# DrorT/demucs

Hardware: NVIDIA B200
Metric: htdemucs audio-seconds separated per second (higher is better)
Workload: dtype f32 (bf16 hi/lo split operands, 3 tcgen05 products, fp32 accumulate)

## Files before the change

### demucs_b200/_lib.py

```python
from __future__ import annotations

import ctypes as C
import os
import subprocess
import typing as tp

HERE = os.path.dirname(os.path.abspath(__file__))
CSRC = os.path.join(HERE, "csrc")
LIB_PATH = os.path.join(HERE, "libdemucs_b200.so")
SOURCES = ["api.cu", "spectral.cu", "gemm_simt.cu", "gemm_tc.cu", "gemm_tc_b16x3.cu", "gemm_tc_b16.cu", "norm.cu", "dconv.cu", "attention.cu", "attention_tc.cu", "attention_b16.cu",
           "ola.cu", "audio.cu", "hdemucs.cu"]
NVCC_FLAGS = ["-gencode", "arch=compute_100a,code=sm_100a", "-lineinfo", "-O3", "-std=c++17",
              "-Xcompiler", "-fPIC", "--use_fast_math=false"]

BD_MAX_TAPS = 9
A_NONE, A_GN_GELU, A_ITEM_AFFINE = 0, 1, 2
ACT_NONE, ACT_GELU, ACT_GLU = 0, 1, 2
MATH_FP32, MATH_TF32, MATH_TF32X3, MATH_BF16X3, MATH_BF16 = 0, 1, 2, 3, 4


class KernelError(RuntimeError):
    pass


class GemmDesc(C.Structure):
    _fields_ = [
        ("M", C.c_int), ("N", C.c_int), ("K", C.c_int),
        ("Cin", C.c_int), ("taps", C.c_int),
        ("I1", C.c_int), ("I0", C.c_int),
        ("m1", C.c_int), ("m0", C.c_int), ("J1", C.c_int), ("J0", C.c_int),
        ("d1", C.c_int * BD_MAX_TAPS), ("d0", C.c_int * BD_MAX_TAPS),
        ("xs_b", C.c_longlong), ("xs_1", C.c_longlong), ("xs_0", C.c_longlong), ("xs_c", C.c_longlong),
        ("x", C.c_void_p), ("w", C.c_void_p), ("bias", C.c_void_p),
        ("a_mode", C.c_int), ("a_stats", C.c_void_p), ("a_stats_stride", C.c_int),
        ("a_gamma", C.c_void_p), ("a_beta", C.c_void_p),
        ("e_stats", C.c_void_p), ("e_gamma", C.c_void_p), ("e_beta", C.c_void_p),
        ("act", C.c_int), ("rowbias", C.c_void_p), ("rowbias_period", C.c_int),
        ("resid", C.c_void_p), ("scale", C.c_void_p), ("addend", C.c_void_p),
        ("out", C.c_void_p), ("os_b", C.c_longlong), ("os_1", C.c_longlong), ("os_0", C.c_longlong),
        ("convt", C.c_int), ("O0", C.c_int), ("oc_split", C.c_int), ("oc_stride", C.c_longlong),
        ("stats_out", C.c_void_p), ("stat_div", C.c_int), ("stat_mul", C.c_int), ("stat_mod", C.c_int),
        ("math", C.c_int), ("w16_hi", C.c_void_p), ("w16_lo", C.c_void_p), ("x_bf16", C.c_int), ("out_bf16", C.c_int),
    ]


_P, _I, _LL, _D, _F = C.c_void_p, C.c_int, C.c_longlong, C.c_double, C.c_float
SIGNATURES: tp.Dict[str, tp.List] = {
    "bd_stft_cac": [_P, _P, _P, _P, _P, _I, _I, _I, _P],
    "bd_finalize_item_norm": [_P, _P, _I, _D, _D, _P],
    "bd_istft_frames": [_P, _P, _P, _P, _P, _I, _I, _I, _P],
    "bd_istft_ola": [_P, _P, _P, _P, _P, _P, _I, _I, _I, _I, _I, _P],
    "bd_ola_combine": [_P, _P, _P, _P, _I, _I, _I, _I, _I, _P],
    "bd_conv_gemm": [C.POINTER(GemmDesc), _P],
    "bd_conv_gemm_arm": [C.POINTER(GemmDesc)],
    "bd_finalize_group_stats": [_P, _P, _I, _D, _P],
    "bd_dconv_tail": [_P, _P, _P, _P, _P, _P, _LL, _I, _LL, _I, _P],
    "bd_encoder_conv0": [_P, _I, _P, _I, _P, _P, _P, _I, _I, _I, _I, _I, _I, _I, _P],
    "bd_dconv_conv3": [_P, _P, _P, _P, _I, _P, _LL, _I, _I, _LL, _I, _I, _I, _P],
    "bd_dconv_expand_stats": [_P, _I, _I, _P, _P, _P, _P, _P, _P, _P, _LL, _I, _LL, _I, _P],
    "bd_dconv_expand_update": [_P, _I, _I, _P, _P, _P, _P, _P, _P, _P, _P, _P, _P, _LL, _I, _LL, _I, _I, _P],
    "bd_gn_gelu_apply": [_P, _P, _P, _P, _LL, _I, _LL, _I, _P],
    "bd_layer_norm": [_P, _P, _P, _P, _P, _I, _LL, _I, _I, _P],
    "bd_attention_bf16": [_P, _P, _P, _P, _I, _I, _I, _I, _I, _I, _I, _I, _P],
    "bd_item_stats": [_P, _P, _I, _LL, _P],
    "bd_group_norm_apply": [_P, _P, _P, _P, _I, _LL, _I, _P],
    "bd_attention_workspace": [_I, _I, _I, _I, _I],
    "bd_attention": [_P, _P, _P, _P, _I, _I, _I, _I, _I, _I, _I, _I, _I, _P, _P],
    "bd_overlap_add": [_P, _P, _P, _I, _I, _I, _I, _I, _I, _I, _LL, _LL, _LL, _LL, _LL, _P, _F, _I, _P],
    "bd_gather_segments": [_P, _P, _I, _I, _LL, _LL, _LL, _I, _I, _I, _I, _I, _P],
    "bd_gn_stats": [_P, _P, _I, _LL, _I, _I, _P],
    "bd_gn_act": [_P, _P, _P, _P, _P, _P, _I, _LL, _LL, _LL, _I, _I, _I, _LL, _P],
    "bd_lstm_frame": [_P, _P, _I, _LL, _I, _I, _I, _I, _P],
    "bd_lstm_unframe_add": [_P, _P, _P, _I, _LL, _I, _I, _I, _I, _P],
    "bd_lstm_bidir": [_P, _P, _P, _P, _I, _I, _I, _P],
    "bd_local_state": [_P, _P, _P, _I, _I, _I, _I, _P],
    "bd_convert_channels": [_P, _P, _I, _I, _I, _LL, _P],
    "bd_resample_frac": [_P, _P, _P, _I, _I, _I, _LL, _LL, _I, _I, _I, _P],
    "bd_absmax": [_P, _P, _LL, _P],
    "bd_clip_pcm": [_P, _P, _I, _LL, _I, _P, _I, _P],
}
VALUE_CALLS = {"bd_attention_workspace"}
EXPORTS = ["bd_last_error", "bd_version"] + list(SIGNATURES)

_lib: tp.Optional[C.CDLL] = None


def build(verbose: bool = False, force: bool = False) -> str:
    import hashlib
    from concurrent.futures import ThreadPoolExecutor
    srcs = [os.path.join(CSRC, s) for s in SOURCES if os.path.exists(os.path.join(CSRC, s))]
    headers = [os.path.join(os.path.dirname(HERE), "include", "demucs_b200.h")]
    headers += sorted(os.path.join(CSRC, f) for f in os.listdir(CSRC) if f.endswith(".cuh"))
    flags = [f for f in NVCC_FLAGS if not f.startswith("--use_fast_math")]
    flags += os.environ.get("BD_NVCC_DEFS", "").split()
    base = hashlib.sha256(" ".join(flags).encode())
    for dep in headers:
        with open(dep, "rb") as f:
            base.update(f.read())
    nvcc = os.environ.get("NVCC", "/usr/local/cuda/bin/nvcc")
    objdir = os.path.join(CSRC, ".obj")
    os.makedirs(objdir, exist_ok=True)
    total = base.copy()
    jobs = []
    for src in srcs:
        d = base.copy()
        with open(src, "rb") as f:
            data = f.read()
        d.update(data)
        total.update(data)
        obj = os.path.join(objdir, os.path.basename(src)[:-3] + ".o")
        jobs.append((src, obj, d.hexdigest()))
    stamp_path = LIB_PATH + ".stamp"
    stamp = total.hexdigest()
    if not force and os.path.exists(LIB_PATH) and os.path.exists(stamp_path):
        with open(stamp_path) as f:
            if f.read().strip() == stamp:
                return LIB_PATH

    def compile_one(job):
        src, obj, digest = job
        if not force and os.path.exists(obj) and os.path.exists(obj + ".stamp"):
            with open(obj + ".stamp") as f:
                if f.read().strip() == digest:
                    return ""
        cmd = [nvcc] + flags + (["-Xptxas=-v"] if verbose else []) + ["-c", "-o", obj, src]
        res = subprocess.run(cmd, capture_output=True, text=True)
        if res.returncode != 0:
            raise KernelError(f"nvcc failed on {src}:\n{res.stdout}\n{res.stderr}")
        with open(obj + ".stamp", "w") as f:
            f.write(digest)
        return res.stderr

    with ThreadPoolExecutor(max_workers=min(len(jobs), os.cpu_count() or 4)) as pool:
        logs = list(pool.map(compile_one, jobs))
    if verbose:
        print("\n".join(logs))
    res = subprocess.run([nvcc] + flags + ["-shared", "-o", LIB_PATH] + [j[1] for j in jobs], capture_output=True, text=True)
    if res.returncode != 0:
        raise KernelError(f"link failed:\n{res.stdout}\n{res.stderr}")
    with open(stamp_path, "w") as f:
        f.write(stamp)
    return LIB_PATH


def lib() -> C.CDLL:
    global _lib
    if _lib is None:
        if not os.path.exists(LIB_PATH):
            raise KernelError(
                f"{LIB_PATH} is missing: run `python -c 'import __graft_entry__ as g; g.build()'` "
                "(demucs_b200 has no CPU or PyTorch fallback path)")
        handle = C.CDLL(LIB_PATH)
        handle.bd_last_error.restype = C.c_char_p
        handle.bd_last_error.argtypes = []
        handle.bd_version.restype = C.c_int
        for name, args in SIGNATURES.items():
            fn = getattr(handle, name)
            fn.restype = C.c_longlong if name in VALUE_CALLS else C.c_int
            fn.argtypes = args
        _lib = handle
    return _lib


TEST_HOOK: tp.Optional[tp.Callable] = None


def call(name: str, *args) -> None:
    if TEST_HOOK is not None:
        return TEST_HOOK(name, *args)
    rc = getattr(lib(), name)(*args)
    if rc != 0:
        raise KernelError(f"{name} failed ({rc}): {lib().bd_last_error().decode()}")


def call_value(name: str, *args) -> int:
    if TEST_HOOK is not None:
        return TEST_HOOK(name, *args)
    return int(getattr(lib(), name)(*args))


def ptr(t) -> tp.Optional[int]:
    return None if t is None else t.data_ptr()
```

### demucs_b200/csrc/gemm_tc.cu

```cuda
#include "gemm_tc_impl.cuh"

int bd_tc_launch_bf16x3(int tbk, int tbn, const bd_gemm_desc& d, const TileGeom& g, int items, cudaStream_t st);
int bd_tc_launch_bf16(int tbk, int tbn, const bd_gemm_desc& d, const TileGeom& g, int items, cudaStream_t st);
int bd_tc_launch_bf16d(int tbk, int tbn, const bd_gemm_desc& d, const TileGeom& g, int items, cudaStream_t st);

namespace {
int pow2_ceil(int v) {
  int p = 1;
  while (p < v) p <<= 1;
  return p;
}
}

bool bd_conv_gemm_tc_eligible(const bd_gemm_desc& d) {
  if (d.a_mode != BD_A_NONE || d.xs_c != 1 || d.m1 != 1) return false;
  if (!(d.m0 == 1 || (d.m0 == 4 && d.J0 % 4 == 0))) return false;
  if (d.Cin % 16 != 0 || d.N < 16 || d.K < 16 || d.M < 128 || d.taps > BD_MAX_TAPS) return false;
  if (d.x_bf16) {
    if (d.math != BD_MATH_BF16 || d.Cin % 64 != 0) return false;
    if (d.xs_0 % 8 != 0 || (d.J1 > 1 && d.xs_1 % 8 != 0) || d.xs_b % 8 != 0) return false;
  }
  if (d.xs_0 % 4 != 0 || (d.J1 > 1 && d.xs_1 % 4 != 0) || d.xs_b % 4 != 0) return false;
  if (((uintptr_t)d.x & 15) || ((uintptr_t)d.w & 15)) return false;
  if (d.math == BD_MATH_BF16X3 || d.math == BD_MATH_BF16) {
    if (!d.w16_hi || ((uintptr_t)d.w16_hi & 15) || d.K % 8 != 0) return false;
    if (d.math == BD_MATH_BF16X3 && (!d.w16_lo || ((uintptr_t)d.w16_lo & 15))) return false;
  }
  if (d.stats_out && d.stat_mod == 1 && !(d.I1 == 1 && d.I0 == d.stat_div)) return false;
  return true;
}

namespace {

TileGeom tile_geometry(const bd_gemm_desc& d) {
  TileGeom g;
  g.R0 = (d.I0 >= 128 || d.I1 == 1) ? 128 : (pow2_ceil(d.I0) > 128 ? 128 : pow2_ceil(d.I0));
  g.R1 = 128 / g.R0;
  g.log2R0 = 0;
  while ((1 << g.log2R0) < g.R0) ++g.log2R0;
  g.blocks0 = (d.I0 + g.R0 - 1) / g.R0;
  g.blocks1 = (d.I1 + g.R1 - 1) / g.R1;
  g.stride4 = d.m0 == 4;
  g.cpb = 0;
  return g;
}

int tile_width(const bd_gemm_desc& d, const TileGeom& g) {
  static const bool wide_ok = getenv("BD_TC_NO_WIDE") == nullptr;
  static const bool wide_x3 = getenv("BD_TC_NO_WIDE_X3") == nullptr;
  const int items = d.M / (d.I0 * d.I1);
  const bool wide = wide_ok && (d.math != BD_MATH_TF32X3 || wide_x3) && d.N % 256 == 0 &&
                    d.K >= 256 && d.out && !d.convt && !d.oc_split && !d.rowbias && !d.addend && !d.e_stats &&
                    (!d.stats_out || d.stat_mod == 1) && bd_epi_vec_ok(d);
  auto wave_eff = [&](int tile_n) {
    const long long t = (long long)items * g.blocks1 * g.blocks0 * ((d.N + tile_n - 1) / tile_n);
    return (double)t / (double)(((t + 147) / 148) * 148);
  };
  if (wide && wave_eff(256) >= wave_eff(128) - 0.05) return 256;
  return d.N <= 16 ? 16 : d.N <= 32 ? 32 : d.N <= 64 ? 64 : 128;
}

}

static int k_block(const bd_gemm_desc& d, int tbn) {
  if (d.x_bf16) return 64;
  if (d.math == BD_MATH_BF16X3 || d.math == BD_MATH_BF16) return d.Cin % 32 == 0 ? 32 : 16;
  return (tbn == 256 || d.math == BD_MATH_TF32X3 || d.Cin % 32 != 0) ? 16 : 32;
}

int bd_conv_gemm_tc_tile(const bd_gemm_desc& d) {
  if (!bd_conv_gemm_tc_eligible(d) || d.M % ((long long)d.I0 * d.I1) != 0) return 0;
  const int tbn = tile_width(d, tile_geometry(d));
  return 1000 * k_block(d, tbn) + tbn;
}

int bd_conv_gemm_tc(const bd_gemm_desc* dp, void* stream, int* handled) {
  const bd_gemm_desc& d = *dp;
  *handled = 0;
  if (!bd_conv_gemm_tc_eligible(d)) return BD_OK;
  BD_REQUIRE(d.act != BD_ACT_GLU || d.N % 2 == 0, "bd_conv_gemm: GLU needs even N");
  BD_REQUIRE(d.M % ((long long)d.I0 * d.I1) == 0, "bd_conv_gemm: M not a multiple of I1*I0");
  TileGeom g = tile_geometry(d);
  const int items = d.M / (d.I0 * d.I1);
  const int tbn = tile_width(d, g);
  const int tbk = k_block(d, tbn);
  g.cpb = d.Cin / tbk;
  const cudaStream_t st = (cudaStream_t)stream;
  int rc;
  switch (d.math) {
    case BD_MATH_BF16X3: rc = bd_tc_launch_bf16x3(tbk, tbn, d, g, items, st); break;
    case BD_MATH_BF16:
      rc = d.x_bf16 ? bd_tc_launch_bf16d(tbk, tbn, d, g, items, st) : bd_tc_launch_bf16(tbk, tbn, d, g, items, st);
      break;
    case BD_MATH_TF32X3:
      rc = tbn == 256 ? launch_tc_persist<16, 256, BD_TC_TF32X3>(d, g, items, st)
                      : launch_tc_width<16, BD_TC_TF32X3>(tbn, d, g, items, st);
      break;
    default:
      rc = tbn == 256 ? launch_tc_persist<16, 256, BD_TC_TF32>(d, g, items, st)
           : tbk == 32 ? launch_tc_width<32, BD_TC_TF32>(tbn, d, g, items, st)
                       : launch_tc_width<16, BD_TC_TF32>(tbn, d, g, items, st);
      break;
  }
  *handled = 1;
  return rc;
}
```

### demucs_b200/csrc/gemm_tc_impl.cuh

```cuda
#pragma once
#include <cuda.h>
#include <stdlib.h>
#include "gemm_epilogue.cuh"

enum { BD_TC_TF32 = 0, BD_TC_TF32X3 = 1, BD_TC_BF16X3 = 2, BD_TC_BF16 = 3, BD_TC_BF16D = 4 };

struct TileGeom {
  int R0, R1;
  int log2R0;
  int blocks0, blocks1;
  int cpb;
  int stride4;
};

namespace {

constexpr int TBM = 128;


struct RowInfo {
  long long obase;
  int i0;
  int rb_row;
  float e_mean, e_rstd;
  int pad0, pad1;
};

constexpr uint32_t kSpinLimit = 1u << 26;

__device__ __forceinline__ uint32_t smem_u32(const void* p) { return (uint32_t)__cvta_generic_to_shared(p); }

__device__ __forceinline__ void mbar_init(uint64_t* bar, uint32_t count) {
  asm volatile("mbarrier.init.shared::cta.b64 [%0], %1;" ::"r"(smem_u32(bar)), "r"(count));
}
__device__ __forceinline__ void mbar_arrive(uint64_t* bar) {
  asm volatile("mbarrier.arrive.shared::cta.b64 _, [%0];" ::"r"(smem_u32(bar)) : "memory");
}
__device__ __forceinline__ void mbar_expect_tx(uint64_t* bar, uint32_t bytes) {
  asm volatile("mbarrier.arrive.expect_tx.shared::cta.b64 _, [%0], %1;" ::"r"(smem_u32(bar)), "r"(bytes) : "memory");
}
__device__ __forceinline__ void mbar_wait(uint64_t* bar, uint32_t parity) {
  uint32_t done = 0, spins = 0;
  while (true) {
    asm volatile(
        "{\n\t.reg .pred p;\n\t"
        "mbarrier.try_wait.parity.shared::cta.b64 p, [%1], %2;\n\t"
        "selp.u32 %0, 1, 0, p;\n\t}"
        : "=r"(done)
        : "r"(smem_u32(bar)), "r"(parity)
        : "memory");
    if (done) return;
    if (++spins > kSpinLimit) __trap();
  }
}
__device__ __forceinline__ void mbar_wait_parked(uint64_t* bar, uint32_t parity) {
  uint32_t done = 0, spins = 0;
  while (true) {
    asm volatile(
        "{\n\t.reg .pred p;\n\t"
        "mbarrier.try_wait.parity.shared::cta.b64 p, [%1], %2, %3;\n\t"
        "selp.u32 %0, 1, 0, p;\n\t}"
        : "=r"(done)
        : "r"(smem_u32(bar)), "r"(parity), "r"(1000)
        : "memory");
    if (done) return;
    if (++spins > kSpinLimit) __trap();
  }
}
__device__ __forceinline__ void mbar_wait_relaxed(uint64_t* bar, uint32_t parity) {
  uint32_t done = 0, spins = 0;
  while (true) {
    asm volatile(
        "{\n\t.reg .pred p;\n\t"
        "mbarrier.try_wait.parity.shared::cta.b64 p, [%1], %2;\n\t"
        "selp.u32 %0, 1, 0, p;\n\t}"
        : "=r"(done)
        : "r"(smem_u32(bar)), "r"(parity)
        : "memory");
    if (done) return;
    __nanosleep(64);
    if (++spins > kSpinLimit) __trap();
  }
}
__device__ __forceinline__ void tma_load_4d(const CUtensorMap* map, uint64_t* bar, void* dst, int c0, int c1, int c2,
                                            int c3) {
  asm volatile(
      "cp.async.bulk.tensor.4d.shared::cluster.global.mbarrier::complete_tx::bytes [%0], [%1, {%3, %4, %5, %6}], [%2];"
      ::"r"(smem_u32(dst)), "l"((uint64_t)map), "r"(smem_u32(bar)), "r"(c0), "r"(c1), "r"(c2), "r"(c3)
      : "memory");
}
__device__ __forceinline__ void tma_load_5d(const CUtensorMap* map, uint64_t* bar, void* dst, int c0, int c1, int c2,
                                            int c3, int c4) {
  asm volatile(
      "cp.async.bulk.tensor.5d.shared::cluster.global.mbarrier::complete_tx::bytes [%0], [%1, {%3, %4, %5, %6, %7}], "
      "[%2];"
      ::"r"(smem_u32(dst)), "l"((uint64_t)map), "r"(smem_u32(bar)), "r"(c0), "r"(c1), "r"(c2), "r"(c3), "r"(c4)
      : "memory");
}
__device__ __forceinline__ void tma_load_2d(const CUtensorMap* map, uint64_t* bar, void* dst, int c0, int c1) {
  asm volatile(
      "cp.async.bulk.tensor.2d.shared::cluster.global.mbarrier::complete_tx::bytes [%0], [%1, {%3, %4}], [%2];"
      ::"r"(smem_u32(dst)), "l"((uint64_t)map), "r"(smem_u32(bar)), "r"(c0), "r"(c1)
      : "memory");
}
__device__ __forceinline__ void tcgen05_commit(uint64_t* bar) {
  asm volatile("tcgen05.commit.cta_group::1.mbarrier::arrive::one.shared::cluster.b64 [%0];" ::"r"(smem_u32(bar))
               : "memory");
}
__device__ __forceinline__ void tcgen05_fence_after() { asm volatile("tcgen05.fence::after_thread_sync;" ::: "memory"); }
__device__ __forceinline__ void tcgen05_fence_before() { asm volatile("tcgen05.fence::before_thread_sync;" ::: "memory"); }

__device__ __forceinline__ void umma_tf32(uint32_t tmem_d, uint64_t adesc, uint64_t bdesc, uint32_t idesc, uint32_t accumulate) {
  asm volatile(
      "{\n\t.reg .pred p;\n\t"
      "setp.ne.b32 p, %4, 0;\n\t"
      "tcgen05.mma.cta_group::1.kind::tf32 [%0], %1, %2, %3, p;\n\t}"
      ::"r"(tmem_d), "l"(adesc), "l"(bdesc), "r"(idesc), "r"(accumulate)
      : "memory");
}

__device__ __forceinline__ void umma_bf16(uint32_t tmem_d, uint64_t adesc, uint64_t bdesc, uint32_t idesc, uint32_t accumulate) {
  asm volatile(
      "{\n\t.reg .pred p;\n\t"
      "setp.ne.b32 p, %4, 0;\n\t"
      "tcgen05.mma.cta_group::1.kind::f16 [%0], %1, %2, %3, p;\n\t}"
      ::"r"(tmem_d), "l"(adesc), "l"(bdesc), "r"(idesc), "r"(accumulate)
      : "memory");
}

template <int TBK>
__device__ __forceinline__ uint64_t make_kmajor_desc(const void* smem) {
  uint64_t desc = (uint64_t)((smem_u32(smem) & 0x3FFFF) >> 4);
  desc |= (uint64_t)((8 * TBK * 4) >> 4) << 32;
  desc |= (uint64_t)1 << 46;
  desc |= (uint64_t)(TBK == 32 ? 2 : 4) << 61;
  return desc;
}
template <int TBK>
__device__ __forceinline__ uint64_t make_kmajor_desc16(const void* smem, int sbo) {
  uint64_t desc = (uint64_t)((smem_u32(smem) & 0x3FFFF) >> 4);
  desc |= (uint64_t)(sbo >> 4) << 32;
  desc |= (uint64_t)1 << 46;
  desc |= (uint64_t)(TBK == 64 ? 2 : TBK == 32 ? 4 : 6) << 61;
  return desc;
}
__host__ __device__ constexpr uint32_t make_idesc_bf16(int M, int N) {
  return (1u << 4) | (1u << 7) | (1u << 10) | ((uint32_t)(N >> 3) << 17) | ((uint32_t)(M >> 4) << 24);
}
__device__ __forceinline__ uint32_t pack_bf16(float a, float b) {
  uint32_t r;
  asm("cvt.rn.bf16x2.f32 %0, %1, %2;" : "=r"(r) : "f"(b), "f"(a));
  return r;
}
__host__ __device__ constexpr uint32_t make_idesc_tf32(int M, int N) {
  return (1u << 4) | (2u << 7) | (2u << 10) | ((uint32_t)(N >> 3) << 17) | ((uint32_t)(M >> 4) << 24);
}

__device__ __forceinline__ void tmem_ld32(uint32_t taddr, uint32_t* r) {
  asm volatile(
      "tcgen05.ld.sync.aligned.32x32b.x32.b32 "
      "{%0, %1, %2, %3, %4, %5, %6, %7, %8, %9, %10, %11, %12, %13, %14, %15, "
      "%16, %17, %18, %19, %20, %21, %22, %23, %24, %25, %26, %27, %28, %29, %30, %31}, [%32];"
      : "=r"(r[0]), "=r"(r[1]), "=r"(r[2]), "=r"(r[3]), "=r"(r[4]), "=r"(r[5]), "=r"(r[6]), "=r"(r[7]), "=r"(r[8]),
        "=r"(r[9]), "=r"(r[10]), "=r"(r[11]), "=r"(r[12]), "=r"(r[13]), "=r"(r[14]), "=r"(r[15]), "=r"(r[16]),
        "=r"(r[17]), "=r"(r[18]), "=r"(r[19]), "=r"(r[20]), "=r"(r[21]), "=r"(r[22]), "=r"(r[23]), "=r"(r[24]),
        "=r"(r[25]), "=r"(r[26]), "=r"(r[27]), "=r"(r[28]), "=r"(r[29]), "=r"(r[30]), "=r"(r[31])
      : "r"(taddr));
  asm volatile("tcgen05.wait::ld.sync.aligned;" ::: "memory");
}

__device__ __forceinline__ float rn_tf32(float x) {
  uint32_t u;
  asm("cvt.rna.tf32.f32 %0, %1;" : "=r"(u) : "f"(x));
  return __uint_as_float(u);
}

__device__ __forceinline__ void tmem_ld16(uint32_t taddr, uint32_t* r) {
  asm volatile(
      "tcgen05.ld.sync.aligned.32x32b.x16.b32 "
      "{%0, %1, %2, %3, %4, %5, %6, %7, %8, %9, %10, %11, %12, %13, %14, %15}, [%16];"
      : "=r"(r[0]), "=r"(r[1]), "=r"(r[2]), "=r"(r[3]), "=r"(r[4]), "=r"(r[5]), "=r"(r[6]), "=r"(r[7]), "=r"(r[8]),
        "=r"(r[9]), "=r"(r[10]), "=r"(r[11]), "=r"(r[12]), "=r"(r[13]), "=r"(r[14]), "=r"(r[15])
      : "r"(taddr));
  asm volatile("tcgen05.wait::ld.sync.aligned;" ::: "memory");
}

__device__ __forceinline__ float sigmoid_fast(float x) {
  float e, r;
  asm("ex2.approx.ftz.f32 %0, %1;" : "=f"(e) : "f"(-1.44269504088896340736f * x));
  asm("rcp.approx.ftz.f32 %0, %1;" : "=f"(r) : "f"(1.0f + e));
  return r;
}
__device__ __forceinline__ float4 lds128(uint32_t a) {
  float4 v;
  asm volatile("ld.shared.v4.f32 {%0, %1, %2, %3}, [%4];" : "=f"(v.x), "=f"(v.y), "=f"(v.z), "=f"(v.w) : "r"(a));
  return v;
}

template <int ACT, bool E, bool RES, bool ROWB, bool CT, int WC, int RB>
__device__ __forceinline__ void epi_fast_rows(const bd_gemm_desc& d, uint32_t stage_s, uint32_t rinfo_s, int lane, int n0w,
                                              float& ssum, float& ssq) {
  constexpr int LDT = WC + 4;
  constexpr int CG = WC / 4 < 32 ? WC / 4 : 32;
  constexpr int RPI = 32 / CG;
  const int cg = lane % CG, rsub = lane / CG;
  const int n = n0w + 4 * cg;
  const bool col_ok = n < d.N;
  const int nc = col_ok ? n : 0;
  const float4 bias = d.bias ? ldg4(d.bias + nc) : make_float4(0.f, 0.f, 0.f, 0.f);
  float4 gam = make_float4(1.f, 1.f, 1.f, 1.f), bet = make_float4(0.f, 0.f, 0.f, 0.f);
  if (E) {
    gam = ldg4(d.e_gamma + nc);
    bet = ldg4(d.e_beta + nc);
  }
  const int no = ACT == BD_ACT_GLU ? nc >> 1 : nc;
  float4 scl = make_float4(1.f, 1.f, 1.f, 1.f);
  if (RES && d.scale) {
    if (ACT == BD_ACT_GLU) {
      const float2 t = ldg2(d.scale + no);
      scl.x = t.x; scl.y = t.y;
    } else {
      scl = ldg4(d.scale + no);
    }
  }
  int rr = 0;
  long long colofs = no;
  if (CT) {
    const int cout = d.N >> 2;
    rr = nc / cout;
    colofs = (long long)rr * d.os_0 + (nc - rr * cout);
    rr -= d.convt == 1 ? 2 : 0;
  }
  const long long outo = colofs;
  const float* resp = RES ? d.resid + colofs : nullptr;
  const float* addp = CT && d.addend ? d.addend + colofs : nullptr;
  const float* rbp = ROWB ? d.rowbias + no : nullptr;
  const int rb_ld = ACT == BD_ACT_GLU ? d.N >> 1 : d.N;
  const uint32_t st_lane = stage_s + (uint32_t)(rsub * LDT + 4 * cg) * 4u;
  const uint32_t ri_lane = rinfo_s + (uint32_t)rsub * 32u;
#pragma unroll 1
  for (int it = 0; it < 32 / RPI; it += RB) {
    long long ob[RB];
    bool ok[RB];
    float mean[RB], rstd[RB];
    float4 res[RB];
#pragma unroll
    for (int u = 0; u < RB; ++u) {
      const uint32_t ra = ri_lane + (uint32_t)((it + u) * RPI) * 32u;
      uint32_t w0, w1, w2, w3;
      asm volatile("ld.shared.v4.u32 {%0, %1, %2, %3}, [%4];" : "=r"(w0), "=r"(w1), "=r"(w2), "=r"(w3) : "r"(ra));
      ob[u] = (long long)(((unsigned long long)w1 << 32) | w0);
      ok[u] = (int)w2 >= 0 && col_ok;
      if (CT) ok[u] = ok[u] && (unsigned)(4 * (int)w2 + rr) < (unsigned)d.O0;
      if (ROWB || CT) res[u] = make_float4(0.f, 0.f, 0.f, 0.f);
      if (ROWB && ok[u]) {
        if (ACT == BD_ACT_GLU) {
          const float2 t = ldg2(rbp + (size_t)w3 * rb_ld);
          res[u].x = t.x; res[u].y = t.y;
        } else {
          res[u] = ldg4(rbp + (size_t)w3 * rb_ld);
        }
      }
      if (CT && addp && ok[u]) res[u] = ldg4(addp + ob[u]);
      if (E) asm volatile("ld.shared.v2.f32 {%0, %1}, [%2];" : "=f"(mean[u]), "=f"(rstd[u]) : "r"(ra + 16));
      if (RES) {
        res[u] = make_float4(0.f, 0.f, 0.f, 0.f);
        if (ok[u]) {
          if (ACT == BD_ACT_GLU) {
            const float2 t = ldg2(resp + ob[u]);
            res[u].x = t.x; res[u].y = t.y;
          } else {
            res[u] = ldg4(resp + ob[u]);
          }
        }
      }
    }
#pragma unroll
    for (int u = 0; u < RB; ++u) {
      float4 v = lds128(st_lane + (uint32_t)((it + u) * RPI * LDT) * 4u);
      v.x += bias.x; v.y += bias.y; v.z += bias.z; v.w += bias.w;
      if (E) {
        v.x = fmaf((v.x - mean[u]) * rstd[u], gam.x, bet.x);
        v.y = fmaf((v.y - mean[u]) * rstd[u], gam.y, bet.y);
        v.z = fmaf((v.z - mean[u]) * rstd[u], gam.z, bet.z);
        v.w = fmaf((v.w - mean[u]) * rstd[u], gam.w, bet.w);
      }
      if (ACT == BD_ACT_GLU) {
        float2 o2 = make_float2(v.x * sigmoid_fast(v.y), v.z * sigmoid_fast(v.w));
        if (ROWB) {
          o2.x += res[u].x;
          o2.y += res[u].y;
        }
        if (RES) {
          o2.x = fmaf(scl.x, o2.x, res[u].x);
          o2.y = fmaf(scl.y, o2.y, res[u].y);
        }
        if (ok[u]) {
          bd_store_out2(d, outo + ob[u], o2);
          ssum += o2.x + o2.y;
          ssq = fmaf(o2.x, o2.x, fmaf(o2.y, o2.y, ssq));
        }
      } else {
        if (ACT == BD_ACT_GELU) {
          v.x = bd_gelu(v.x); v.y = bd_gelu(v.y); v.z = bd_gelu(v.z); v.w = bd_gelu(v.w);
        }
        if (RES) {
          v.x = fmaf(scl.x, v.x, res[u].x); v.y = fmaf(scl.y, v.y, res[u].y);
          v.z = fmaf(scl.z, v.z, res[u].z); v.w = fmaf(scl.w, v.w, res[u].w);
        }
        if (ROWB || CT) {
          v.x += res[u].x; v.y += res[u].y; v.z += res[u].z; v.w += res[u].w;
        }
        if (ok[u]) {
          bd_store_out4(d, outo + ob[u], v);
          ssum += (v.x + v.y) + (v.z + v.w);
          ssq = fmaf(v.x, v.x, fmaf(v.y, v.y, fmaf(v.z, v.z, fmaf(v.w, v.w, ssq))));
        }
      }
    }
  }
}

__device__ __forceinline__ int epi_fast_id(const bd_gemm_desc& d, bool vec, bool row_stats) {
  if (!vec || row_stats || !d.out || d.oc_split) return -1;
  const bool e = d.e_stats != nullptr, r = d.resid != nullptr;
  if (d.convt) return (d.act == BD_ACT_GELU && !e && !r && !d.rowbias) ? 6 : -1;
  if (d.addend) return -1;
  if (d.rowbias) return (d.act == BD_ACT_GLU && !e && !r) ? 5 : -1;
  if (d.act == BD_ACT_NONE && !e) return r ? 1 : 0;
  if (d.act == BD_ACT_GELU && !e && !r) return 2;
  if (d.act == BD_ACT_GLU && !e && !r) return 3;
  if (d.act == BD_ACT_GLU && e && r) return 4;
  return -1;
}

#ifndef BD_TC_EPI_GROUPS
#define BD_TC_EPI_GROUPS 4
#endif
template <int TBK, int TBN, int MODE>
struct PCfg {
  static constexpr bool kX3 = MODE == BD_TC_TF32X3;
  static constexpr bool kB16 = MODE == BD_TC_BF16X3 || MODE == BD_TC_BF16 || MODE == BD_TC_BF16D;
  static constexpr bool kDirect = MODE == BD_TC_BF16D;
  static constexpr bool kSplit = MODE != BD_TC_TF32 && !kDirect;
  static constexpr int kBParts = MODE == BD_TC_BF16X3 ? 2 : 1;
  static constexpr int kPGroups = (MODE == BD_TC_TF32X3 || MODE == BD_TC_BF16X3) ? 2 : BD_TC_EPI_GROUPS;
  static constexpr int kSplitWarp0 = kB16 ? 2 : 4;
  static constexpr int kSplitWarps = MODE == BD_TC_BF16 ? 2 : 4;
  static constexpr int kEpiWarp0 = kSplit ? kSplitWarp0 + kSplitWarps : 4;
  static constexpr int kThreads = 32 * kEpiWarp0 + 128 * kPGroups;
  static constexpr int kTileBytesA = TBM * TBK * (kDirect ? 2 : 4);
  static constexpr int kTileBytesB = kB16 ? TBN * TBK * 2 : TBN * TBK * 4;
  static constexpr int kStageBytesA = (kX3 ? 2 : 1) * kTileBytesA;
  static constexpr int kStageBytesB = (kX3 ? 2 : kBParts) * kTileBytesB;
  static constexpr int kTxBytes = kTileBytesA + (kB16 ? kBParts : 1) * kTileBytesB;
  static constexpr bool kTileSplit = TBN <= 32;
  static constexpr int kNAcc = kTileSplit ? kPGroups : 2;
  static constexpr int kHalves = TBN > 128 ? 2 : 1;
  static constexpr int kWarpCols = kTileSplit ? TBN : (TBN / kHalves) / kPGroups;
  static constexpr int kStagingBytes = 4 * kPGroups * 32 * (kWarpCols + 4) * 4;
  static constexpr int kTailBytes = 512 + 128 * kPGroups * 32;
  static constexpr int kBudget = 227 * 1024 - 1024 - kTailBytes - kStagingBytes;
  static constexpr int kStagesRaw = kBudget / (kStageBytesA + kStageBytesB);
  static constexpr int kStages = kStagesRaw > (kTileSplit ? 16 : 8) ? (kTileSplit ? 16 : 8) : kStagesRaw;
  static constexpr int kSmemBytes = kStages * (kStageBytesA + kStageBytesB) + kStagingBytes + 1024 + kTailBytes;
  static constexpr int kTmemCols = kNAcc * TBN < 32 ? 32 : kNAcc * TBN;
};

template <int TBK, int TBN, int MODE>
__global__ void __launch_bounds__((PCfg<TBK, TBN, MODE>::kThreads), 1) conv_gemm_tc_persist_kernel(const __grid_constant__ CUtensorMap map_a,
                                                                            const __grid_constant__ CUtensorMap map_b,
                                                                            const __grid_constant__ CUtensorMap map_b_lo,
                                                                            const bd_gemm_desc d, const TileGeom g,
                                                                            int ntiles, int ntn) {
  using C_ = PCfg<TBK, TBN, MODE>;
  constexpr bool X3 = C_::kX3, B16 = C_::kB16, SPLIT = C_::kSplit;
  constexpr int kPGroups = C_::kPGroups;
  constexpr int kTileBytesA = C_::kTileBytesA, kTileBytesB = C_::kTileBytesB;
  constexpr int kStages = C_::kStages, kStageBytesA = C_::kStageBytesA, kStageBytesB = C_::kStageBytesB;
  constexpr int kTmemCols = C_::kTmemCols;
  constexpr int WC = C_::kWarpCols;
  constexpr int CW = WC < 32 ? WC : 32;
  extern __shared__ uint8_t smem_raw[];
  uint8_t* smem = reinterpret_cast<uint8_t*>(((uintptr_t)smem_raw + 1023) & ~(uintptr_t)1023);
  uint8_t* sA = smem;
  uint8_t* sB = smem + kStages * kStageBytesA;
  float* staging = reinterpret_cast<float*>(sB + kStages * kStageBytesB);
  uint64_t* full_bar = reinterpret_cast<uint64_t*>(reinterpret_cast<uint8_t*>(staging) + C_::kStagingBytes);
  uint64_t* empty_bar = full_bar + kStages;
  constexpr int kNAcc = C_::kNAcc;
  constexpr bool kTileSplit = C_::kTileSplit;
  constexpr int NH = C_::kHalves;
  uint64_t* tmem_full = empty_bar + kStages;
  uint64_t* tmem_empty = tmem_full + kNAcc;
  uint64_t* conv_bar = tmem_empty + kNAcc;
  uint32_t* tmem_slot = reinterpret_cast<uint32_t*>(conv_bar + kStages);

  const int warp = threadIdx.x >> 5, lane = threadIdx.x & 31;
  const int nkb = d.taps * g.cpb;

  if (threadIdx.x == 0) {
    for (int s = 0; s < kStages; ++s) {
      mbar_init(&full_bar[s], 1);
      mbar_init(&empty_bar[s], 1);
      mbar_init(&conv_bar[s], 32 * C_::kSplitWarps);
    }
    for (int a = 0; a < kNAcc; ++a) {
      mbar_init(&tmem_full[a], 1);
      mbar_init(&tmem_empty[a], kTileSplit ? 4 : 4 * kPGroups);
    }
    asm volatile("fence.mbarrier_init.release.cluster;" ::: "memory");
  }
  if (warp == 1) {
    asm volatile("tcgen05.alloc.cta_group::1.sync.aligned.shared::cta.b32 [%0], %1;" ::"r"(smem_u32(tmem_slot)),
                 "r"(kTmemCols));
    asm volatile("tcgen05.relinquish_alloc_permit.cta_group::1.sync.aligned;" ::);
  }
  tcgen05_fence_before();
  __syncthreads();
  tcgen05_fence_after();
  const uint32_t tmem_base = *tmem_slot;

  auto decode = [&](int tile, int& b, int& i0s, int& i1s, int& n0) {
    const int nb = tile % ntn;
    int r = tile / ntn;
    const int blk0 = r % g.blocks0;
    r /= g.blocks0;
    const int blk1 = r % g.blocks1;
    b = r / g.blocks1;
    i0s = blk0 * g.R0;
    i1s = blk1 * g.R1;
    n0 = nb * TBN;
  };

  if (warp == 0) {
    if (lane == 0) {
      long long kbg = 0;
      for (int tile = blockIdx.x; tile < ntiles; tile += gridDim.x) {
        int b, i0s, i1s, n0;
        decode(tile, b, i0s, i1s, n0);
        int tap = 0, cb = 0;
        for (int kb = 0; kb < nkb; ++kb, ++kbg) {
          const int s = (int)(kbg % kStages);
          const uint32_t ph = (uint32_t)((kbg / kStages) & 1);
          mbar_wait_parked(&empty_bar[s], ph ^ 1);
          mbar_expect_tx(&full_bar[s], C_::kTxBytes);
          if (g.stride4) {
            const int d0 = d.d0[tap];
            tma_load_5d(&map_a, &full_bar[s], sA + s * kStageBytesA, cb * TBK, d0 & 3, i0s + (d0 >> 2), i1s + d.d1[tap], b);
          } else {
            tma_load_4d(&map_a, &full_bar[s], sA + s * kStageBytesA, cb * TBK, i0s + d.d0[tap], i1s + d.d1[tap], b);
          }
          tma_load_2d(&map_b, &full_bar[s], sB + s * kStageBytesB, tap * d.Cin + cb * TBK, n0);
          if constexpr (MODE == BD_TC_BF16X3)
            tma_load_2d(&map_b_lo, &full_bar[s], sB + s * kStageBytesB + kTileBytesB, tap * d.Cin + cb * TBK, n0);
          if (++cb == g.cpb) {
            cb = 0;
            ++tap;
          }
        }
      }
    }
  } else if (warp == 1) {
    if (lane == 0) {
      constexpr uint32_t idesc = B16 ? make_idesc_bf16(TBM, TBN) : make_idesc_tf32(TBM, TBN);
      long long kbg = 0;
      int tcount = 0;
      for (int tile = blockIdx.x; tile < ntiles; tile += gridDim.x, ++tcount) {
        const int a = tcount % kNAcc;
        mbar_wait_parked(&tmem_empty[a], (uint32_t)(((tcount / kNAcc) & 1) ^ 1));
        tcgen05_fence_after();
        const uint32_t acc = tmem_base + (uint32_t)(a * TBN);
        for (int kb = 0; kb < nkb; ++kb, ++kbg) {
          const int s = (int)(kbg % kStages);
          const uint32_t ph = (uint32_t)((kbg / kStages) & 1);
          mbar_wait_parked(SPLIT ? &conv_bar[s] : &full_bar[s], ph);
          tcgen05_fence_after();
          if constexpr (B16) {
            const uint64_t a_hi = make_kmajor_desc16<TBK>(sA + s * kStageBytesA, C_::kDirect ? 8 * TBK * 2 : 8 * TBK * 4);
            const uint64_t a_lo = make_kmajor_desc16<TBK>(sA + s * kStageBytesA + 8 * TBK * 2, 8 * TBK * 4);
            const uint64_t b_hi = make_kmajor_desc16<TBK>(sB + s * kStageBytesB, 8 * TBK * 2);
            const uint64_t b_lo = make_kmajor_desc16<TBK>(sB + s * kStageBytesB + kTileBytesB, 8 * TBK * 2);
#pragma unroll
            for (int k = 0; k < TBK / 16; ++k) {
              if constexpr (MODE == BD_TC_BF16X3) {
                umma_bf16(acc, a_lo + 2 * k, b_hi + 2 * k, idesc, (kb | k) != 0);
                umma_bf16(acc, a_hi + 2 * k, b_lo + 2 * k, idesc, 1);
                umma_bf16(acc, a_hi + 2 * k, b_hi + 2 * k, idesc, 1);
              } else {
                umma_bf16(acc, a_hi + 2 * k, b_hi + 2 * k, idesc, (kb | k) != 0);
              }
            }
          } else {
          const uint64_t adesc = make_kmajor_desc<TBK>(sA + s * kStageBytesA);
          const uint64_t bdesc = make_kmajor_desc<TBK>(sB + s * kStageBytesB);
#pragma unroll
          for (int k = 0; k < TBK / 8; ++k) {
            if constexpr (X3) {
              const uint64_t alo = make_kmajor_desc<TBK>(sA + s * kStageBytesA + kTileBytesA);
              const uint64_t blo = make_kmajor_desc<TBK>(sB + s * kStageBytesB + kTileBytesB);
              umma_tf32(acc, alo + 2 * k, bdesc + 2 * k, idesc, (kb | k) != 0);
              umma_tf32(acc, adesc + 2 * k, blo + 2 * k, idesc, 1);
              umma_tf32(acc, adesc + 2 * k, bdesc + 2 * k, idesc, 1);
            } else {
              umma_tf32(acc, adesc + 2 * k, bdesc + 2 * k, idesc, (kb | k) != 0);
            }
          }
          }
          tcgen05_commit(&empty_bar[s]);
        }
        tcgen05_commit(&tmem_full[a]);
      }
    }
  } else if (SPLIT && warp >= C_::kSplitWarp0 && warp < C_::kSplitWarp0 + C_::kSplitWarps) {
    const int et = threadIdx.x - 32 * C_::kSplitWarp0;
    long long kbg = 0;
    if constexpr (B16) {
      constexpr int RB = TBK * 4, RH = TBK * 2;
      constexpr int GB = 8 * RB;
      constexpr int SW = C_::kSplitWarps;
      constexpr int NG = (TBM / 8) / SW;
      const int sw = warp - C_::kSplitWarp0, r = lane >> 2, q = lane & 3;
      const int xin = (r * RB >> 7) & (RB / 16 - 1);
      const int xout = (r * RH >> 7) & (RH / 16 - 1);
      (void)et;
      for (int tile = blockIdx.x; tile < ntiles; tile += gridDim.x) {
        for (int kb = 0; kb < nkb; ++kb, ++kbg) {
          const int s = (int)(kbg % kStages);
          mbar_wait(&full_bar[s], (uint32_t)((kbg / kStages) & 1));
          uint8_t* base = sA + s * kStageBytesA;
#pragma unroll
          for (int i0 = 0; i0 < NG; i0 += 4) {
          float4 v[4][TBK == 32 ? 2 : 1];
#pragma unroll
          for (int i = 0; i < 4; ++i) {
            const uint8_t* gp = base + (sw + SW * (i0 + i)) * GB + r * RB;
            if constexpr (TBK == 32) {
              v[i][0] = *reinterpret_cast<const float4*>(gp + (((2 * q) ^ xin) << 4));
              v[i][1] = *reinterpret_cast<const float4*>(gp + (((2 * q + 1) ^ xin) << 4));
            } else {
              v[i][0] = *reinterpret_cast<const float4*>(gp + ((q ^ xin) << 4));
            }
          }
          __syncwarp();
#pragma unroll
          for (int i = 0; i < 4; ++i) {
            uint8_t* gp = base + (sw + SW * (i0 + i)) * GB + r * RH;
            uint32_t hi[TBK == 32 ? 4 : 2], lo[TBK == 32 ? 4 : 2];
#pragma unroll
            for (int j = 0; j < (TBK == 32 ? 2 : 1); ++j) {
              const float4 x = v[i][j];
              const uint32_t h0 = pack_bf16(x.x, x.y), h1 = pack_bf16(x.z, x.w);
              hi[2 * j] = h0;
              hi[2 * j + 1] = h1;
              lo[2 * j] = lo[2 * j + 1] = 0u;
              if constexpr (MODE == BD_TC_BF16X3) {
                lo[2 * j] = pack_bf16(x.x - __uint_as_float(h0 << 16), x.y - __uint_as_float(h0 & 0xffff0000u));
                lo[2 * j + 1] = pack_bf16(x.z - __uint_as_float(h1 << 16), x.w - __uint_as_float(h1 & 0xffff0000u));
              }
            }
            if constexpr (TBK == 32) {
              uint8_t* dst = gp + ((q ^ xout) << 4);
              *reinterpret_cast<uint4*>(dst) = make_uint4(hi[0], hi[1], hi[2], hi[3]);
              if constexpr (MODE == BD_TC_BF16X3) *reinterpret_cast<uint4*>(dst + 8 * RH) = make_uint4(lo[0], lo[1], lo[2], lo[3]);
            } else {
              uint8_t* dst = gp + (((q >> 1) ^ xout) << 4) + ((q & 1) << 3);
              *reinterpret_cast<uint2*>(dst) = make_uint2(hi[0], hi[1]);
              if constexpr (MODE == BD_TC_BF16X3) *reinterpret_cast<uint2*>(dst + 8 * RH) = make_uint2(lo[0], lo[1]);
            }
          }
          }
          asm volatile("fence.proxy.async.shared::cta;" ::: "memory");
          mbar_arrive(&conv_bar[s]);
        }
      }
    } else {
    for (int tile = blockIdx.x; tile < ntiles; tile += gridDim.x) {
      for (int kb = 0; kb < nkb; ++kb, ++kbg) {
        const int s = (int)(kbg % kStages);
        mbar_wait(&full_bar[s], (uint32_t)((kbg / kStages) & 1));
        auto split = [&](uint8_t* base, int tile_bytes) {
          float4* hi = reinterpret_cast<float4*>(base);
          float4* lo = reinterpret_cast<float4*>(base + tile_bytes);
#pragma unroll 4
          for (int i = et; i < tile_bytes / 16; i += 128) {
            const float4 x = hi[i];
            const float4 h = make_float4(rn_tf32(x.x), rn_tf32(x.y), rn_tf32(x.z), rn_tf32(x.w));
            hi[i] = h;
            lo[i] = make_float4(x.x - h.x, x.y - h.y, x.z - h.z, x.w - h.w);
          }
        };
        split(sA + s * kStageBytesA, kTileBytesA);
        split(sB + s * kStageBytesB, kTileBytesB);
        asm volatile("fence.proxy.async.shared::cta;" ::: "memory");
        mbar_arrive(&conv_bar[s]);
      }
    }
    }
  } else if (warp >= C_::kEpiWarp0) {
    const int quarter = warp & 3, ew = warp - C_::kEpiWarp0, grp = ew >> 2;
    const int cbase = kTileSplit ? 0 : grp * WC;
    const bool row_stats = d.stats_out && d.stat_mod != 1;
    const bool vec = bd_epi_vec_ok(d);
    const int fast = epi_fast_id(d, vec, row_stats);
    constexpr int LDT = WC + 4;
    float* stage = staging + (size_t)ew * 32 * LDT;
    RowInfo* rinfo = reinterpret_cast<RowInfo*>(((uintptr_t)(tmem_slot + 4) + 31) & ~(uintptr_t)31) + ew * 32;
    int tcount = 0;
    for (int tile = blockIdx.x; tile < ntiles; tile += gridDim.x, ++tcount) {
      if (kTileSplit && tcount % kPGroups != grp) continue;
      int b, i0s, i1s, n0;
      decode(tile, b, i0s, i1s, n0);
      const int a = tcount % kNAcc;
      const int r = quarter * 32 + lane;
      const int i0 = i0s + (r & (g.R0 - 1)), i1 = i1s + (r >> g.log2R0);
      const bool row_ok = i0 < d.I0 && i1 < d.I1;
      const long long m = ((long long)b * d.I1 + i1) * d.I0 + i0;
      EpiRow er;
      er.obase = 0; er.i0 = 0; er.rb_row = 0; er.e_mean = 0.f; er.e_rstd = 1.f;
      if (row_ok) {
        er.i0 = i0;
        er.obase = (long long)b * d.os_b + (long long)i1 * d.os_1 +
                   (long long)(d.convt ? 4 * i0 - (d.convt == 1 ? 2 : 0) : i0) * d.os_0;
        if (d.rowbias) er.rb_row = (int)((unsigned)m % (unsigned)d.rowbias_period);
        if (d.e_stats) {
          const int sl = bd_stat_slab(d, m);
          er.e_mean = __ldg(d.e_stats + 2 * (size_t)sl);
          er.e_rstd = __ldg(d.e_stats + 2 * (size_t)sl + 1);
        }
      }
      const int my_slab = (d.stats_out && row_ok) ? bd_stat_slab(d, m) : -1;
      float ssum = 0.f, ssq = 0.f;
      if (d.resid && row_ok && !d.convt && !d.oc_split) {
        const int c0 = n0 + cbase;
        if (c0 < d.N) {
          const float* pf = d.resid + er.obase + (d.act == BD_ACT_GLU ? c0 >> 1 : c0);
          asm volatile("prefetch.global.L2 [%0];" ::"l"(pf));
        }
      }
      for (int half = 0; half < NH; ++half) {
      const int n0h = n0 + 128 * half;
      if (half == 0) {
        mbar_wait_relaxed(&tmem_full[a], (uint32_t)((tcount / kNAcc) & 1));
        tcgen05_fence_after();
      } else {
        __syncwarp();
      }
      const bool last_half = half == NH - 1;
      const uint32_t acc = tmem_base + (uint32_t)(a * TBN + 128 * half + cbase) + ((uint32_t)(quarter * 32) << 16);
      if (vec) {
        rinfo[lane].obase = er.obase;
        rinfo[lane].i0 = row_ok ? er.i0 : -1;
        rinfo[lane].rb_row = er.rb_row;
        rinfo[lane].e_mean = er.e_mean;
        rinfo[lane].e_rstd = er.e_rstd;
        for (int c0 = 0; c0 < WC; c0 += CW) {
          if (n0h + cbase + c0 >= d.N) break;
          uint32_t v[CW];
          if constexpr (CW == 32) tmem_ld32(acc + c0, v); else tmem_ld16(acc + c0, v);
#pragma unroll
          for (int j = 0; j < CW; j += 4)
            *reinterpret_cast<float4*>(stage + lane * LDT + c0 + j) =
                make_float4(__uint_as_float(v[j]), __uint_as_float(v[j + 1]), __uint_as_float(v[j + 2]),
                            __uint_as_float(v[j + 3]));
        }
        tcgen05_fence_before();
        __syncwarp();
        if (lane == 0 && last_half) mbar_arrive(&tmem_empty[a]);
        if (fast >= 0) {
          const uint32_t st_s = smem_u32(stage), ri_s = smem_u32(rinfo);
          const int n0w = n0h + cbase;
          constexpr int FRB = kPGroups >= 4 ? 2 : 4;
          switch (fast) {
            case 0: epi_fast_rows<BD_ACT_NONE, false, false, false, false, WC, FRB>(d, st_s, ri_s, lane, n0w, ssum, ssq); break;
            case 1: epi_fast_rows<BD_ACT_NONE, false, true, false, false, WC, FRB>(d, st_s, ri_s, lane, n0w, ssum, ssq); break;
            case 2: epi_fast_rows<BD_ACT_GELU, false, false, false, false, WC, FRB>(d, st_s, ri_s, lane, n0w, ssum, ssq); break;
            case 3: epi_fast_rows<BD_ACT_GLU, false, false, false, false, WC, FRB>(d, st_s, ri_s, lane, n0w, ssum, ssq); break;
            case 4: epi_fast_rows<BD_ACT_GLU, true, true, false, false, WC, FRB>(d, st_s, ri_s, lane, n0w, ssum, ssq); break;
            case 5: epi_fast_rows<BD_ACT_GLU, false, false, true, false, WC, FRB>(d, st_s, ri_s, lane, n0w, ssum, ssq); break;
            default: epi_fast_rows<BD_ACT_GELU, false, false, false, true, WC, FRB>(d, st_s, ri_s, lane, n0w, ssum, ssq); break;
          }
          __syncwarp();
        } else {
        constexpr int CG = WC / 4 < 32 ? WC / 4 : 32;
        constexpr int RPI = 32 / CG;
        constexpr int RB = kPGroups >= 4 ? 2 : 4;
        const int cg = lane % CG, rsub = lane / CG;
        const int n = n0h + cbase + 4 * cg;
        const bool col_ok = n < d.N;
        EpiCol ecol;
        if (col_ok) ecol = bd_epi_cols4(d, n);
        for (int it = 0; it < 32 / RPI; it += RB) {
          EpiRow row[RB];
          EpiMem mem[RB];
          bool ok[RB];
#pragma unroll
          for (int u = 0; u < RB; ++u) {
            const int rloc = (it + u) * RPI + rsub;
            const uint32_t ra = smem_u32(&rinfo[rloc]);
            uint32_t w0, w1, w2, w3, w4, w5;
            asm volatile("ld.shared.v4.u32 {%0, %1, %2, %3}, [%4];" : "=r"(w0), "=r"(w1), "=r"(w2), "=r"(w3) : "r"(ra));
            asm volatile("ld.shared.v2.u32 {%0, %1}, [%2];" : "=r"(w4), "=r"(w5) : "r"(ra + 16));
            row[u].obase = (long long)(((unsigned long long)w1 << 32) | w0);
            row[u].i0 = (int)w2;
            row[u].rb_row = (int)w3;
            row[u].e_mean = __uint_as_float(w4);
            row[u].e_rstd = __uint_as_float(w5);
            ok[u] = row[u].i0 >= 0 && col_ok;
            if (ok[u]) mem[u] = bd_epi_fetch4(d, row[u], ecol);
          }
#pragma unroll
          for (int u = 0; u < RB; ++u) {
            const int rloc = (it + u) * RPI + rsub;
            float rs = 0.f, rq = 0.f;
            if (ok[u]) {
              const float4 acc4 = *reinterpret_cast<const float4*>(stage + rloc * LDT + 4 * cg);
              bd_epi_finish4(d, row[u], ecol, acc4, mem[u], rs, rq);
            }
            if (row_stats) {
              __syncwarp();
              *reinterpret_cast<float2*>(stage + rloc * LDT + 2 * cg) = make_float2(rs, rq);
            } else {
              ssum += rs;
              ssq += rq;
            }
          }
        }
        if (row_stats) {
          __syncwarp();
          float rs = 0.f, rq = 0.f;
#pragma unroll
          for (int c = 0; c < CG; ++c) {
            const float2 t = *reinterpret_cast<const float2*>(stage + lane * LDT + 2 * c);
            rs += t.x;
            rq += t.y;
          }
          if (my_slab >= 0) {
            atomicAdd(&d.stats_out[2 * (size_t)my_slab], (double)rs);
            atomicAdd(&d.stats_out[2 * (size_t)my_slab + 1], (double)rq);
          }
        }
        __syncwarp();
        }
      } else {
        for (int c0 = 0; c0 < WC; c0 += CW) {
          if (n0h + cbase + c0 >= d.N) break;
          uint32_t v[CW];
          if constexpr (CW == 32) tmem_ld32(acc + c0, v); else tmem_ld16(acc + c0, v);
          if (row_ok) {
#pragma unroll
            for (int j = 0; j < CW; ++j) {
              const int n = n0h + cbase + c0 + j;
              if (n < d.N) {
                float st;
                if (bd_epi_apply(d, er, n, __uint_as_float(v[j]), __uint_as_float(v[(j + 1) % CW]), st)) {
                  ssum += st;
                  ssq = fmaf(st, st, ssq);
                }
              }
            }
          }
        }
        tcgen05_fence_before();
        __syncwarp();
        if (lane == 0 && last_half) mbar_arrive(&tmem_empty[a]);
        if (row_stats && row_ok) {
          atomicAdd(&d.stats_out[2 * (size_t)my_slab], (double)ssum);
          atomicAdd(&d.stats_out[2 * (size_t)my_slab + 1], (double)ssq);
        }
      }
      }
      if (d.stats_out && d.stat_mod == 1) {
        const double ds = bd_warp_sum_d((double)ssum), dq = bd_warp_sum_d((double)ssq);
        if (lane == 0) {
          const int sl = bd_stat_slab(d, (long long)b * d.I1 * d.I0 + i0s);
          atomicAdd(&d.stats_out[2 * (size_t)sl], ds);
          atomicAdd(&d.stats_out[2 * (size_t)sl + 1], dq);
        }
      }
    }
  }
  tcgen05_fence_before();
  __syncthreads();
  if (warp == 1) {
    tcgen05_fence_after();
    asm volatile("tcgen05.dealloc.cta_group::1.sync.aligned.b32 %0, %1;" ::"r"(tmem_base), "r"(kTmemCols));
  }
}

typedef CUresult (*EncodeTiledFn)(CUtensorMap*, CUtensorMapDataType, cuuint32_t, void*, const cuuint64_t*,
                                  const cuuint64_t*, const cuuint32_t*, const cuuint32_t*, CUtensorMapInterleave,
                                  CUtensorMapSwizzle, CUtensorMapL2promotion, CUtensorMapFloatOOBfill);

EncodeTiledFn get_encode_fn() {
  static EncodeTiledFn fn = nullptr;
  if (!fn) {
    void* p = nullptr;
    cudaDriverEntryPointQueryResult q;
    if (cudaGetDriverEntryPoint("cuTensorMapEncodeTiled", &p, cudaEnableDefault, &q) != cudaSuccess ||
        q != cudaDriverEntryPointSuccess)
      return nullptr;
    fn = (EncodeTiledFn)p;
  }
  return fn;
}

bool encode(CUtensorMap* map, const void* base, int rank, const cuuint64_t* gdim, const cuuint64_t* gstride_bytes,
            const cuuint32_t* box, int row_bytes, bool bf16 = false) {
  EncodeTiledFn enc = get_encode_fn();
  if (!enc) return false;
  cuuint32_t estr[5] = {1, 1, 1, 1, 1};
  const CUtensorMapSwizzle sw = row_bytes == 128 ? CU_TENSOR_MAP_SWIZZLE_128B
                                : row_bytes == 64 ? CU_TENSOR_MAP_SWIZZLE_64B : CU_TENSOR_MAP_SWIZZLE_32B;
  return enc(map, bf16 ? CU_TENSOR_MAP_DATA_TYPE_BFLOAT16 : CU_TENSOR_MAP_DATA_TYPE_FLOAT32, rank, (void*)base, gdim,
             gstride_bytes, box, estr, CU_TENSOR_MAP_INTERLEAVE_NONE, sw, CU_TENSOR_MAP_L2_PROMOTION_L2_128B,
             CU_TENSOR_MAP_FLOAT_OOB_FILL_NONE) == CUDA_SUCCESS;
}

template <int TBK, int TBN, int MODE>
int launch_tc_persist(const bd_gemm_desc& d, const TileGeom& g, int items, cudaStream_t st) {
  using C_ = PCfg<TBK, TBN, MODE>;
  alignas(64) CUtensorMap map_a, map_b, map_b_lo;
  const long long s0 = d.xs_0, s1 = d.J1 > 1 ? d.xs_1 : s0 * d.J0, sb = items > 1 ? d.xs_b : s1 * d.J1;
  constexpr int ES = C_::kDirect ? 2 : 4;
  cuuint64_t adim[5] = {(cuuint64_t)d.Cin, (cuuint64_t)d.J0, (cuuint64_t)d.J1, (cuuint64_t)items, 1};
  cuuint64_t astr[4] = {(cuuint64_t)s0 * ES, (cuuint64_t)s1 * ES, (cuuint64_t)sb * ES, 0};
  cuuint32_t abox[5] = {(cuuint32_t)TBK, (cuuint32_t)g.R0, (cuuint32_t)g.R1, 1, 1};
  int arank = 4;
  if (g.stride4) {
    arank = 5;
    adim[1] = 4; adim[2] = (cuuint64_t)d.J0 / 4; adim[3] = (cuuint64_t)d.J1; adim[4] = (cuuint64_t)items;
    astr[0] = (cuuint64_t)s0 * ES; astr[1] = (cuuint64_t)s0 * 4 * ES; astr[2] = (cuuint64_t)s1 * ES; astr[3] = (cuuint64_t)sb * ES;
    abox[1] = 1; abox[2] = (cuuint32_t)g.R0; abox[3] = (cuuint32_t)g.R1; abox[4] = 1;
  }
  cuuint64_t bdim[2] = {(cuuint64_t)d.K, (cuuint64_t)d.N};
  cuuint32_t bbox[2] = {(cuuint32_t)TBK, (cuuint32_t)TBN};
  bool ok = encode(&map_a, d.x, arank, adim, astr, abox, TBK * ES, C_::kDirect);
  if constexpr (C_::kB16) {
    cuuint64_t bstr[1] = {(cuuint64_t)d.K * 2};
    ok = ok && encode(&map_b, d.w16_hi, 2, bdim, bstr, bbox, TBK * 2, true);
    ok = ok && encode(&map_b_lo, MODE == BD_TC_BF16X3 ? d.w16_lo : d.w16_hi, 2, bdim, bstr, bbox, TBK * 2, true);
  } else {
    cuuint64_t bstr[1] = {(cuuint64_t)d.K * 4};
    ok = ok && encode(&map_b, d.w, 2, bdim, bstr, bbox, TBK * 4);
    map_b_lo = map_b;
  }
  if (!ok) {
    bd_set_error("bd_conv_gemm_tc: cuTensorMapEncodeTiled failed (M=%d N=%d K=%d Cin=%d J0=%d J1=%d)", d.M, d.N, d.K,
                 d.Cin, d.J0, d.J1);
    return BD_ERR_CUDA;
  }
  static int sms_of[64] = {0};
  int dev = 0;
  cudaGetDevice(&dev);
  if (dev < 0 || dev >= 64) {
    bd_set_error("bd_conv_gemm_tc: device ordinal %d out of range", dev);
    return BD_ERR_ARG;
  }
  if (!sms_of[dev]) {
    cudaError_t e = cudaFuncSetAttribute(conv_gemm_tc_persist_kernel<TBK, TBN, MODE>,
                                         cudaFuncAttributeMaxDynamicSharedMemorySize, C_::kSmemBytes);
    if (e != cudaSuccess) {
      bd_set_error("bd_conv_gemm_tc: cudaFuncSetAttribute: %s", cudaGetErrorString(e));
      return BD_ERR_CUDA;
    }
    int n = 0;
    cudaDeviceGetAttribute(&n, cudaDevAttrMultiProcessorCount, dev);
    sms_of[dev] = n;
  }
  const int sms = sms_of[dev];
  const int ntn = (d.N + TBN - 1) / TBN;
  const long long ntiles = (long long)items * g.blocks1 * g.blocks0 * ntn;
  const int grid = (int)(ntiles < sms ? ntiles : sms);
  conv_gemm_tc_persist_kernel<TBK, TBN, MODE><<<grid, C_::kThreads, C_::kSmemBytes, st>>>(map_a, map_b, map_b_lo, d, g,
                                                                                         (int)ntiles, ntn);
  return bd_check_launch("conv_gemm_tc_persist_kernel");
}

template <int TBK, int MODE>
int launch_tc_width(int tbn, const bd_gemm_desc& d, const TileGeom& g, int items, cudaStream_t st) {
  switch (tbn) {
    case 16: return launch_tc_persist<TBK, 16, MODE>(d, g, items, st);
    case 32: return launch_tc_persist<TBK, 32, MODE>(d, g, items, st);
    case 64: return launch_tc_persist<TBK, 64, MODE>(d, g, items, st);
    case 128: return launch_tc_persist<TBK, 128, MODE>(d, g, items, st);
    default: break;
  }
  bd_set_error("bd_conv_gemm_tc: no kernel for tile width %d", tbn);
  return BD_ERR_ARG;
}

}
```

### demucs_b200/engine.py

```python
from __future__ import annotations

import ctypes as C
import math
import typing as tp

import numpy as np
import torch

from . import _lib
from ._lib import GemmDesc, call, ptr
from .config import HTDemucsConfig
from .weights import check_state_dict

MODES = ("fp32", "tf32", "tf32x3", "strict", "bf16")
_GEMM_MATH = {"fp32": _lib.MATH_FP32, "tf32": _lib.MATH_TF32, "tf32x3": _lib.MATH_TF32X3, "strict": _lib.MATH_BF16X3,
              "bf16": _lib.MATH_BF16}
_ATTN_MATH = dict(_GEMM_MATH)


def _interleave_glu(w: torch.Tensor) -> torch.Tensor:
    half = w.shape[0] // 2
    return torch.stack([w[:half], w[half:]], dim=1).reshape(w.shape).contiguous()


def _sin_embedding_1d(length: int, dim: int, max_period: float) -> torch.Tensor:
    pos = torch.arange(length, dtype=torch.float32)[:, None]
    half = dim // 2
    k = torch.arange(half, dtype=torch.float32)[None, :]
    phase = pos / (max_period ** (k / (half - 1)))
    return torch.cat([torch.cos(phase), torch.sin(phase)], dim=-1)


def _sin_embedding_2d(dim: int, height: int, width: int, max_period: float) -> torch.Tensor:
    half = dim // 2
    div = torch.exp(torch.arange(0.0, half, 2) * -(math.log(max_period) / half))
    pw = torch.arange(0.0, width)[:, None] * div[None, :]
    ph = torch.arange(0.0, height)[:, None] * div[None, :]
    pe = torch.zeros(width, height, dim)
    pe[:, :, 0:half:2] = torch.sin(pw)[:, None, :]
    pe[:, :, 1:half:2] = torch.cos(pw)[:, None, :]
    pe[:, :, half::2] = torch.sin(ph)[None, :, :]
    pe[:, :, half + 1::2] = torch.cos(ph)[None, :, :]
    return pe.reshape(width * height, dim)


def conv_w(w):
    w = w.detach().float()
    co, ci = w.shape[:2]
    return w.reshape(co, ci, -1).permute(0, 2, 1).reshape(co, -1)


def convtr_w(w):
    w = w.detach().float()
    ci, co = w.shape[:2]
    w = w.reshape(ci, co, 2, 4)
    return w.permute(3, 1, 2, 0).reshape(4 * co, 2 * ci)


def convtr_w3(w):
    w = w.detach().float()
    ci, co = w.shape[:2]
    w = w.reshape(ci, co, 8)
    out = torch.zeros(4, co, 3, ci)
    for s_ in range(4):
        out[s_, :, 1] = w[:, :, s_ + 2].t()
        if s_ <= 1:
            out[s_, :, 0] = w[:, :, s_ + 6].t()
        else:
            out[s_, :, 2] = w[:, :, s_ - 2].t()
    return out.reshape(4 * co, 3 * ci)


def pack_dconv(put, packed, state, prefix: str, depth: int, tc_forms: bool, idx=(0, 1, 3, 4, 6)) -> None:
    i_c3, i_n1, i_c1, i_n2, i_ls = idx
    for d in range(depth):
        p = f"{prefix}.dconv.layers.{d}"
        put(f"{p}.w1", conv_w(state[f"{p}.{i_c3}.weight"]))
        put(f"{p}.b1", state[f"{p}.{i_c3}.bias"])
        put(f"{p}.g1", state[f"{p}.{i_n1}.weight"])
        put(f"{p}.be1", state[f"{p}.{i_n1}.bias"])
        put(f"{p}.w2", _interleave_glu(conv_w(state[f"{p}.{i_c1}.weight"])))
        put(f"{p}.b2", _interleave_glu(state[f"{p}.{i_c1}.bias"].detach().float()))
        put(f"{p}.g2", _interleave_glu(state[f"{p}.{i_n2}.weight"].detach().float()))
        put(f"{p}.be2", _interleave_glu(state[f"{p}.{i_n2}.bias"].detach().float()))
        put(f"{p}.scale", state[f"{p}.{i_ls}.scale"])
        put(f"{p}.w2t", packed[f"{p}.w2"].cpu().t())
        if tc_forms:
            hid = state[f"{p}.{i_c3}.weight"].shape[0]
            hp = (hid + 15) // 16 * 16

            def pad_rows(t):
                t = t.detach().float()
                return torch.cat([t, t.new_zeros((hp - hid,) + tuple(t.shape[1:]))], 0)
            put(f"{p}.w1p", pad_rows(packed[f"{p}.w1"].cpu()))
            put(f"{p}.b1p", pad_rows(state[f"{p}.{i_c3}.bias"]))
            put(f"{p}.g1p", pad_rows(state[f"{p}.{i_n1}.weight"]))
            put(f"{p}.be1p", pad_rows(state[f"{p}.{i_n1}.bias"]))
            put(f"{p}.w2p", pad_rows(packed[f"{p}.w2"].cpu().t()).t())


class PackedWeights:

    def __init__(self, cfg: HTDemucsConfig, state: tp.Mapping[str, torch.Tensor], device, tc_forms: bool = False):
        check_state_dict(cfg, state)
        self.t: tp.Dict[str, torch.Tensor] = {}
        dev = device

        def put(name, tensor):
            self.t[name] = tensor.detach().to(device=dev, dtype=torch.float32).contiguous()

        def dconv(prefix):
            pack_dconv(put, self.t, state, prefix, cfg.dconv_depth, tc_forms)

        for i in range(cfg.depth):
            for name in ("encoder", "tencoder"):
                p = f"{name}.{i}"
                put(f"{p}.conv.w", conv_w(state[f"{p}.conv.weight"]))
                put(f"{p}.conv.b", state[f"{p}.conv.bias"])
                put(f"{p}.rewrite.w", _interleave_glu(conv_w(state[f"{p}.rewrite.weight"])))
                put(f"{p}.rewrite.b", _interleave_glu(state[f"{p}.rewrite.bias"].detach().float()))
                if cfg.dconv_mode & 1:
                    dconv(p)
            for name in ("decoder", "tdecoder"):
                p = f"{name}.{i}"
                put(f"{p}.rewrite.w", _interleave_glu(conv_w(state[f"{p}.rewrite.weight"])))
                put(f"{p}.rewrite.b", _interleave_glu(state[f"{p}.rewrite.bias"].detach().float()))
                put(f"{p}.conv_tr.w", convtr_w(state[f"{p}.conv_tr.weight"]))
                if tc_forms:
                    put(f"{p}.conv_tr.w3", convtr_w3(state[f"{p}.conv_tr.weight"]))
                put(f"{p}.conv_tr.b", state[f"{p}.conv_tr.bias"].detach().float().repeat(4))
                if cfg.dconv_mode & 2:
                    dconv(p)
        if cfg.freq_emb:
            put("freq_emb", cfg.freq_emb * cfg.emb_scale * state["freq_emb.embedding.weight"].detach().float())
        if cfg.bottom_channels:
            for n in ("channel_upsampler", "channel_downsampler", "channel_upsampler_t", "channel_downsampler_t"):
                put(f"{n}.w", state[f"{n}.weight"].detach().float().squeeze(-1))
                put(f"{n}.b", state[f"{n}.bias"])
        if cfg.t_layers > 0:
            for k, v in state.items():
                if k.startswith("crosstransformer."):
                    put(k, v)

    def __getitem__(self, k: str) -> torch.Tensor:
        return self.t[k]

    def nbytes(self) -> int:
        return sum(v.numel() * 4 for v in self.t.values())


class Engine:

    def __init__(self, cfg: HTDemucsConfig, state: tp.Mapping[str, torch.Tensor], device="cuda", mode: str = "fp32"):
        cfg.validate()
        if mode not in MODES:
            raise ValueError(f"mode must be one of {MODES}")
        self.cfg = cfg
        self.mode = mode
        self.device = torch.device(device)
        if self.device.type != "cuda" and _lib.TEST_HOOK is None:
            raise _lib.KernelError("demucs_b200 runs on CUDA devices only (there is no CPU path)")
        _lib.lib()
        self.W = PackedWeights(cfg, state, self.device, tc_forms=(mode != "fp32"))
        k = np.arange(cfg.nfft, dtype=np.float64)
        self.window = torch.from_numpy((0.5 - 0.5 * np.cos(2 * np.pi * k / cfg.nfft)).astype(np.float32)).to(self.device)
        tw = np.stack([np.cos(2 * np.pi * k / cfg.nfft), -np.sin(2 * np.pi * k / cfg.nfft)], axis=1)
        self.twiddle = torch.from_numpy(tw.astype(np.float32)).to(self.device).contiguous()
        self.single_pass = mode in ("tf32", "bf16")
        self.thin_math = {"tf32": _lib.MATH_TF32, "bf16": _lib.MATH_BF16, "tf32x3": _lib.MATH_TF32X3,
                          "strict": _lib.MATH_BF16X3}.get(mode)
        self._w16_cache: tp.Dict[tp.Tuple, tp.Tuple[torch.Tensor, torch.Tensor]] = {}
        self._bufs: tp.Dict[tp.Tuple, tp.Dict[str, torch.Tensor]] = {}
        self._pos: tp.Dict[tp.Tuple, torch.Tensor] = {}
        self.launches = 0
        self._prof: tp.Optional[list] = None

    def _stream(self) -> int:
        if self.device.type != "cuda":
            return 0
        return torch.cuda.current_stream(self.device).cuda_stream

    MAX_BUFFER_SETS = 6

    def _buf(self, key, name: str, numel: int, dtype=torch.float32, zero=False) -> torch.Tensor:
        pool = self._bufs.pop(key, None)
        if pool is None:
            while len(self._bufs) >= self.MAX_BUFFER_SETS:
                self._bufs.pop(next(iter(self._bufs)))
            pool = {}
        self._bufs[key] = pool
        t = pool.get(name)
        if t is None or t.numel() < numel or t.dtype != dtype:
            t = (torch.zeros if zero else torch.empty)(int(numel), dtype=dtype, device=self.device)
            pool[name] = t
        return t[:numel]

    def _k(self, name: str, *args, flops: float = 0.0, nbytes: float = 0.0, label: tp.Optional[str] = None,
           detail: str = "", kernels: int = 1) -> None:
        self.launches += kernels
        if self._prof is None:
            self._call(name, *args)
            return
        e0, e1 = torch.cuda.Event(enable_timing=True), torch.cuda.Event(enable_timing=True)
        e0.record()
        self._call(name, *args)
        e1.record()
        self._prof.append((label or name, e0, e1, flops, nbytes, detail))

    def _call(self, name: str, *args) -> None:
        try:
            if self.device.type != "cuda" and _lib.TEST_HOOK is None:
                raise _lib.KernelError("demucs_b200 runs on CUDA devices only (there is no CPU path)")
            _lib.call(name, *args)
        except Exception:
            self._bufs.clear()
            raise

    def _w16(self, w: torch.Tensor) -> tp.Tuple[torch.Tensor, torch.Tensor]:
        key = (w.data_ptr(), tuple(w.shape))
        got = self._w16_cache.get(key)
        if got is None:
            w = w.contiguous()
            hi = w.to(torch.bfloat16)
            lo = (w - hi.float()).to(torch.bfloat16)
            got = (hi.contiguous(), lo.contiguous(), w)
            self._w16_cache[key] = got
        return got[0], got[1]

    def _gemm(self, *, M, N, Cin, x, w, out, taps=((0, 0),), I1=1, I0=None, m1=1, m0=1, J1=1, J0=None,
              xs=(0, 0, None, 1), os_=(0, 0, None), bias=None, a_mode=_lib.A_NONE, a_stats=None,
              a_stats_stride=0, a_gamma=None, a_beta=None, act=_lib.ACT_NONE, rowbias=None, rowbias_period=0,
              resid=None, scale=None, addend=None, convt=0, O0=0, stats_out=None, stat=(0, 0, 0),
              e_stats=None, e_gamma=None, e_beta=None, oc_split=0, oc_stride=0, tc=True, xf=False, x16=False,
              out16=False) -> None:
        d = GemmDesc()
        I0 = M if I0 is None else I0
        d.M, d.N, d.K, d.Cin, d.taps = M, N, len(taps) * Cin, Cin, len(taps)
        d.I1, d.I0, d.m1, d.m0, d.J1, d.J0 = I1, I0, m1, m0, J1, (I0 if J0 is None else J0)
        for i, (a, b) in enumerate(taps):
            d.d1[i], d.d0[i] = a, b
        n_out = N // 2 if act == _lib.ACT_GLU else (N // 4 if convt else N)
        d.xs_b, d.xs_1, d.xs_0, d.xs_c = xs[0], xs[1], (Cin if xs[2] is None else xs[2]), xs[3]
        d.os_b, d.os_1, d.os_0 = os_[0], os_[1], (n_out if os_[2] is None else os_[2])
        d.x, d.w, d.bias = ptr(x), ptr(w), ptr(bias)
        d.a_mode, d.a_stats, d.a_stats_stride = a_mode, ptr(a_stats), a_stats_stride
        d.a_gamma, d.a_beta = ptr(a_gamma), ptr(a_beta)
        d.e_stats, d.e_gamma, d.e_beta = ptr(e_stats), ptr(e_gamma), ptr(e_beta)
        d.act, d.rowbias, d.rowbias_period = act, ptr(rowbias), rowbias_period
        d.resid, d.scale, d.addend = ptr(resid), ptr(scale), ptr(addend)
        d.out, d.convt, d.O0 = ptr(out), convt, O0
        d.oc_split, d.oc_stride = oc_split, oc_stride
        d.stats_out = ptr(stats_out)
        d.stat_div, d.stat_mul, d.stat_mod = stat
        d.math = _lib.MATH_FP32 if not tc else (_lib.MATH_TF32 if (self.mode == "bf16" and not xf) else _GEMM_MATH[self.mode])
        if d.math in (_lib.MATH_BF16X3, _lib.MATH_BF16) and Cin % 16 == 0 and _lib.TEST_HOOK is None:
            hi, lo = self._w16(w)
            d.w16_hi, d.w16_lo = ptr(hi), ptr(lo)
        d.x_bf16, d.out_bf16 = int(x16), int(out16)
        K = len(taps) * Cin
        rows_in = (M // (I1 * I0)) * d.J1 * d.J0
        nbytes = (2.0 if x16 else 4.0) * rows_in * Cin + (2.0 if d.w16_hi else 4.0) * N * K + \
            (2.0 if out16 else 4.0) * (M * (N if convt else n_out) if out is not None else 0)
        nbytes += 4.0 * M * n_out * ((resid is not None) + (addend is not None))
        arm = "simt"
        tile = 128 if N > 64 else 64 if N > 32 else 32 if (N > 16 or act == _lib.ACT_GLU) else 16
        if d.math != _lib.MATH_FP32 and _lib.TEST_HOOK is None:
            code = _lib.lib().bd_conv_gemm_arm(C.byref(d))
            if code:
                arm, tile = "tc", f"{code // 1000},{code % 1000}"
        self._k("bd_conv_gemm", C.byref(d), self._stream(), flops=2.0 * M * N * K, nbytes=nbytes,
                label=f"conv_gemm_{arm}<{tile}>",
                detail=f"M={M} N={N} K={K} taps={len(taps)} act={act} a={a_mode} stats={int(stats_out is not None)}")

    def _dconv(self, key, prefix: str, x: torch.Tensor, B: int, T: int, Fr: int, C_: int, tag: str):
        cfg, W = self.cfg, self.W
        hid = int(C_ / cfg.dconv_comp)
        M = B * T * Fr
        slabs = B * Fr
        stat = (T * Fr, Fr, Fr)
        tc = self.mode != "fp32"
        narrow = tc and hid == 6 and C_ == 48
        hp = 8 if narrow else ((hid + 15) // 16 * 16 if tc else hid)
        h = self._buf(key, f"dconv_h{tag}", M * hp)
        sums = self._buf(key, f"dconv_sums{tag}", 2 * slabs, torch.float64, zero=True)
        mr1 = self._buf(key, f"dconv_mr1{tag}", 2 * slabs)
        mr2 = self._buf(key, f"dconv_mr2{tag}", 2 * slabs)
        sfx = "p" if tc else ""
        for dd in range(cfg.dconv_depth):
            p = f"{prefix}.dconv.layers.{dd}"
            dil = 2 ** dd
            if narrow:
                self._k("bd_dconv_conv3", ptr(x), ptr(W[f"{p}.w1"]), ptr(W[f"{p}.b1"]), ptr(h), hp, ptr(sums), M, C_, hid,
                        T * Fr, Fr, dil, self.thin_math, self._stream(), flops=2.0 * M * hid * 3 * C_, nbytes=4.0 * M * (C_ + hid),
                        label="dconv_conv3_mma", detail=f"M={M} C={C_} hid={hid} dil={dil}")
            elif Fr == 1:
                geo = dict(taps=((0, -dil), (0, 0), (0, dil)), I1=1, I0=T, J1=1, J0=T,
                           xs=(T * C_, 0, C_, 1), os_=(T * hp, 0, hp))
            else:
                geo = dict(taps=((-dil, 0), (0, 0), (dil, 0)), I1=T, I0=Fr, J1=T, J0=Fr,
                           xs=(T * Fr * C_, Fr * C_, C_, 1), os_=(T * Fr * hp, Fr * hp, hp))
            if not narrow:
                self._gemm(M=M, N=hp, Cin=C_, x=x, w=W[f"{p}.w1{sfx}"], bias=W[f"{p}.b1{sfx}"], out=h,
                           stats_out=sums, stat=stat, tc=tc, **geo)
            self._k("bd_finalize_group_stats", ptr(sums), ptr(mr1), slabs, float(T * hid), self._stream())
            gram = self._buf(key, f"dconv_gram{tag}.{hid}", (slabs + 1) * (hid * hid + hid) + hid + 2, dtype=torch.float64,
                             zero=True)
            self._k("bd_dconv_expand_stats", ptr(h), hp, hid, ptr(mr1), ptr(W[f"{p}.g1"]), ptr(W[f"{p}.be1"]),
                    ptr(W[f"{p}.w2t"]), ptr(W[f"{p}.b2"]), ptr(sums), ptr(gram), M, C_, T * Fr, Fr, self._stream(),
                    nbytes=4.0 * M * hid, flops=4.0 * M * hid * C_, label="dconv_expand_stats",
                    detail=f"M={M} C={C_} hid={hid}", kernels=2)
            self._k("bd_finalize_group_stats", ptr(sums), ptr(mr2), slabs, float(T * 2 * C_), self._stream())
            if tc and hid >= (48 if self.single_pass else 24):
                self._k("bd_gn_gelu_apply", ptr(h), ptr(mr1), ptr(W[f"{p}.g1p"]), ptr(W[f"{p}.be1p"]), M, hp, T * Fr, Fr,
                        self._stream(), nbytes=8.0 * M * hp, label="bd_gn_gelu_apply")
                self._gemm(M=M, N=2 * C_, Cin=hp, x=h, w=W[f"{p}.w2p"], bias=W[f"{p}.b2"], e_stats=mr2,
                           e_gamma=W[f"{p}.g2"], e_beta=W[f"{p}.be2"], act=_lib.ACT_GLU, resid=x, scale=W[f"{p}.scale"],
                           out=x, stat=stat)
                continue
            self._k("bd_dconv_expand_update", ptr(h), hp, hid, ptr(mr1), ptr(W[f"{p}.g1"]), ptr(W[f"{p}.be1"]),
                    ptr(W[f"{p}.w2t"]), ptr(W[f"{p}.b2"]), ptr(mr2), ptr(W[f"{p}.g2"]), ptr(W[f"{p}.be2"]),
                    ptr(W[f"{p}.scale"]), ptr(x), M, C_, T * Fr, Fr,
                    self.thin_math if tc else _lib.MATH_FP32, self._stream(),
                    nbytes=4.0 * M * (hid + 2 * C_), flops=4.0 * M * hid * C_, label="dconv_expand_update",
                    detail=f"M={M} C={C_} hid={hid}")

    def _attention_block(self, key, x, kv_src, p: str, attn: str, B: int, Tq: int, Tk: int, tag: str):
        W, D, H = self.W, self.cfg.transformer_dim, self.cfg.t_heads
        Win, bin_ = W[f"{p}.{attn}.in_proj_weight"], W[f"{p}.{attn}.in_proj_bias"]
        if self.mode == "bf16":
            return self._attention_block_bf16(key, x, kv_src, Win, bin_, B, Tq, Tk, tag)
        att = self._buf(key, f"att{tag}", B * Tq * D)
        nws = _lib.call_value("bd_attention_workspace", B, H, Tq, Tk, self._math())
        ws = self._buf(key, f"att_ws{tag}", nws) if nws else None
        label = "attention_simt" if self.mode == "fp32" else "attention_tc"
        nk = {_lib.MATH_FP32: 1, _lib.MATH_TF32: 2, _lib.MATH_TF32X3: 4, _lib.MATH_BF16X3: 4, _lib.MATH_BF16: 4}[self._math()]
        if kv_src is None:
            qkv = self._buf(key, f"qkv{tag}", B * Tq * 3 * D)
            self._gemm(M=B * Tq, N=3 * D, Cin=D, x=x, w=Win, bias=bin_, out=qkv, xf=True)
            self._k("bd_attention", ptr(qkv), qkv.data_ptr() + 4 * D, qkv.data_ptr() + 8 * D, ptr(att),
                    B, H, Tq, Tq, 3 * D, 3 * D, 3 * D, D, self._math(), ptr(ws), self._stream(),
                    flops=4.0 * B * Tq * Tq * D, nbytes=4.0 * B * Tq * D * 4, label=label, kernels=nk)
        else:
            q = self._buf(key, f"q{tag}", B * Tq * D)
            kv = self._buf(key, f"kv{tag}", B * Tk * 2 * D)
            self._gemm(M=B * Tq, N=D, Cin=D, x=x, w=Win[:D], bias=bin_[:D], out=q, xf=True)
            self._gemm(M=B * Tk, N=2 * D, Cin=D, x=kv_src, w=Win[D:], bias=bin_[D:], out=kv, xf=True)
            self._k("bd_attention", ptr(q), ptr(kv), kv.data_ptr() + 4 * D, ptr(att),
                    B, H, Tq, Tk, D, 2 * D, 2 * D, D, self._math(), ptr(ws), self._stream(),
                    flops=4.0 * B * Tq * Tk * D, nbytes=4.0 * B * (2 * Tq + 2 * Tk) * D, label=label, kernels=nk)
        return att

    def _attention_block_bf16(self, key, x, kv_src, Win, bin_, B: int, Tq: int, Tk: int, tag: str):
        D, H = self.cfg.transformer_dim, self.cfg.t_heads
        bf = torch.bfloat16
        att = self._buf(key, f"att16{tag}", B * Tq * D, bf)
        if kv_src is None:
            qkv = self._buf(key, f"qkv16{tag}", B * Tq * 3 * D, bf)
            self._gemm(M=B * Tq, N=3 * D, Cin=D, x=x, w=Win, bias=bin_, out=qkv, xf=True, x16=True, out16=True)
            self._k("bd_attention_bf16", ptr(qkv), qkv.data_ptr() + 2 * D, qkv.data_ptr() + 4 * D, ptr(att),
                    B, H, Tq, Tq, 3 * D, 3 * D, 3 * D, D, self._stream(),
                    flops=4.0 * B * Tq * Tq * D, nbytes=2.0 * B * Tq * D * 4, label="attention_tc")
        else:
            q = self._buf(key, f"q16{tag}", B * Tq * D, bf)
            kv = self._buf(key, f"kv16{tag}", B * Tk * 2 * D, bf)
            self._gemm(M=B * Tq, N=D, Cin=D, x=x, w=Win[:D], bias=bin_[:D], out=q, xf=True, x16=True, out16=True)
            self._gemm(M=B * Tk, N=2 * D, Cin=D, x=kv_src, w=Win[D:], bias=bin_[D:], out=kv, xf=True, x16=True, out16=True)
            self._k("bd_attention_bf16", ptr(q), ptr(kv), kv.data_ptr() + 2 * D, ptr(att),
                    B, H, Tq, Tk, D, 2 * D, 2 * D, D, self._stream(),
                    flops=4.0 * B * Tq * Tk * D, nbytes=2.0 * B * (2 * Tq + 2 * Tk) * D, label="attention_tc")
        return att

    def _math(self) -> int:
        return _ATTN_MATH[self.mode]

    def _ln(self, x, y, p: str, M: int, pos=None, period=0):
        D = self.cfg.transformer_dim
        y16 = y.dtype == torch.bfloat16
        self._k("bd_layer_norm", ptr(x), ptr(y), ptr(self.W[f"{p}.weight"]), ptr(self.W[f"{p}.bias"]),
                ptr(pos), period, M, D, int(y16), self._stream(), nbytes=(6.0 if y16 else 8.0) * M * D)

    def _transformer_layer(self, key, x, other_normed, p: str, cross: bool, B: int, T: int, Tk: int, tag: str):
        W, D, Hd = self.W, self.cfg.transformer_dim, self.cfg.ffn_dim
        M = B * T
        b16 = self.mode == "bf16"
        adt = torch.bfloat16 if b16 else torch.float32
        ln = self._buf(key, f"ln{tag}", M * D, adt)
        self._ln(x, ln, f"{p}.norm1", M)
        att = self._attention_block(key, ln, other_normed if cross else None, p,
                                    "cross_attn" if cross else "self_attn", B, T, Tk, tag)
        a = "cross_attn" if cross else "self_attn"
        self._gemm(M=M, N=D, Cin=D, x=att, w=W[f"{p}.{a}.out_proj.weight"], bias=W[f"{p}.{a}.out_proj.bias"],
                   out=x, resid=x, scale=W[f"{p}.gamma_1.scale"], xf=True, x16=b16)
        self._ln(x, ln, f"{p}.norm3" if cross else f"{p}.norm2", M)
        hbuf = self._buf(key, f"ffn{tag}", M * Hd, adt)
        self._gemm(M=M, N=Hd, Cin=D, x=ln, w=W[f"{p}.linear1.weight"], bias=W[f"{p}.linear1.bias"], out=hbuf,
                   act=_lib.ACT_GELU, xf=True, x16=b16, out16=b16)
        sums = self._buf(key, f"no_sums{tag}", 2 * B, torch.float64, zero=True)
        mr = self._buf(key, f"no_mr{tag}", 2 * B)
        self._gemm(M=M, N=D, Cin=Hd, x=hbuf, w=W[f"{p}.linear2.weight"], bias=W[f"{p}.linear2.bias"], out=x,
                   resid=x, scale=W[f"{p}.gamma_2.scale"], I1=1, I0=T, J0=T, xs=(T * Hd, 0, Hd, 1),
                   os_=(T * D, 0, D), stats_out=sums, stat=(T, 1, 1), xf=True, x16=b16)
        self._k("bd_finalize_group_stats", ptr(sums), ptr(mr), B, float(T * D), self._stream())
        self._k("bd_group_norm_apply", ptr(x), ptr(mr), ptr(W[f"{p}.norm_out.weight"]),
                ptr(W[f"{p}.norm_out.bias"]), B, T, D, self._stream(), nbytes=8.0 * B * T * D)

    @torch.no_grad()
    def forward(self, mix: torch.Tensor, taps: tp.Optional[dict] = None, out: tp.Optional[torch.Tensor] = None) -> torch.Tensor:
        try:
            if self.device.type == "cuda":
                with torch.cuda.device(self.device):
                    return self._forward(mix, taps, out)
            return self._forward(mix, taps, out)
        except BaseException:
            self._bufs.clear()
            raise

    @torch.no_grad()
    def forward_core(self, mag: torch.Tensor, mix: torch.Tensor) -> tp.Tuple[torch.Tensor, torch.Tensor]:
        try:
            if self.device.type == "cuda":
                with torch.cuda.device(self.device):
                    return self._forward(mix, None, None, mag=mag)
            return self._forward(mix, None, None, mag=mag)
        except BaseException:
            self._bufs.clear()
            raise

    def _forward(self, mix: torch.Tensor, taps: tp.Optional[dict], out_buf: tp.Optional[torch.Tensor], mag=None):
        cfg, W = self.cfg, self.W
        if mix.dim() != 3 or mix.shape[1] != cfg.audio_channels:
            raise ValueError(f"expected mix of shape [B, {cfg.audio_channels}, L], got {tuple(mix.shape)}")
        if mix.device != self.device or mix.dtype != torch.float32:
            raise ValueError("mix must be a float32 tensor on the engine's device")
        B, A, L0 = mix.shape
        L = cfg.segment_length
        if L0 > L:
            raise ValueError(f"Given length {L0} is longer than training length {L}")
        key = (B, L)
        st = self._stream()
        if L0 < L:
            padded = self._buf(key, "mix_padded", B * A * L).view(B, A, L)
            padded.zero_()
            padded[..., :L0].copy_(mix)
            mix = padded
        mix = mix.contiguous()
        S = cfg.n_sources
        T = cfg.frames(L)
        chans = cfg.enc_channels

        def tp(n):
            return (n + 3) // 4 * 4

        def tap(name, t, fmt):
            if taps is None:
                return
            if fmt == "f":
                taps[name] = t.permute(0, 3, 2, 1).clone()
            else:
                taps[name] = t.permute(0, 2, 1).clone()

        spec = self._buf(key, "spec", B * T * 2048 * 4)
        stats = self._buf(key, "item_stats", 4 * B, torch.float64)
        norm = self._buf(key, "item_norm", 8 * B)
        stats.zero_()
        if mag is None:
            self._k("bd_stft_cac", ptr(mix), ptr(self.window), ptr(self.twiddle), ptr(spec), ptr(stats), B, A, L, st,
                    nbytes=4.0 * B * (A * L + T * 2048 * 4), flops=2.5 * 4096 * 12 * 2 * B * T)
        else:
            if L0 != L or tuple(mag.shape) != (B, 2 * A, 2048, T) or mag.device != self.device or mag.dtype != torch.float32:
                raise ValueError(f"forward_core expects mag [B, {2 * A}, 2048, {T}] and mix [B, {A}, {L}] (float32, on "
                                 f"the engine's device), got {tuple(mag.shape)} and {tuple(mix.shape)}")
            spec.view(B, T, 2048, 2 * A).copy_(mag.permute(0, 3, 2, 1))
            pair = self._buf(key, "core_stats", 4 * B, torch.float64)
            pair.zero_()
            self._k("bd_item_stats", ptr(spec), ptr(pair), B, 2 * A * 2048 * T, st, nbytes=4.0 * spec.numel())
            self._k("bd_item_stats", ptr(mix), pair.data_ptr() + 16 * B, B, A * L, st, nbytes=4.0 * mix.numel())
            stats.view(B, 4)[:, :2].copy_(pair[:2 * B].view(B, 2))
            stats.view(B, 4)[:, 2:].copy_(pair[2 * B:].view(B, 2))
        self._k("bd_finalize_item_norm", ptr(stats), ptr(norm), B, float(4 * 2048 * T), float(A * L), st)
        tap("stft", spec.view(B, T, 2048, 4), "f")

        tl = cfg.time_lengths(L)
        saved, saved_t = [], []
        xf, Fin, Cin = spec, 2048, 2 * A
        xt, Cin_t = mix, A
        for i, Cc in enumerate(chans):
            Tin, Tout = tl[i], tl[i + 1]
            y = self._buf(key, "y_t", B * Tout * Cc)
            first = i == 0
            Tin_p = Tin if first else tp(Tin)
            conv0 = first and self.mode != "fp32" and Cc == 48 and A == 2
            if conv0:
                self._k("bd_encoder_conv0", ptr(xt), 1, norm.data_ptr() + 16, 8, ptr(W[f"tencoder.{i}.conv.w"]),
                        ptr(W[f"tencoder.{i}.conv.b"]), ptr(y), B, 1, Tout, L, A, Cc, self.thin_math, self._stream(),
                        flops=2.0 * B * Tout * Cc * 8 * A, nbytes=4.0 * B * (A * L + Tout * Cc), label="encoder_conv0_mma",
                        detail=f"M={B * Tout} cin={A}")
            else:
              self._gemm(M=B * Tout, N=Cc, Cin=Cin_t, x=xt, w=W[f"tencoder.{i}.conv.w"], bias=W[f"tencoder.{i}.conv.b"],
                       out=y, taps=tuple((0, k - 2) for k in range(8)), I1=1, I0=Tout, m0=4, J1=1, J0=Tin_p,
                       xs=(A * L, 0, 1, L) if first else (Tin_p * Cin_t, 0, Cin_t, 1), os_=(Tout * Cc, 0, Cc),
                       a_mode=_lib.A_ITEM_AFFINE if first else _lib.A_NONE,
                       a_stats=norm[4:] if first else None, a_stats_stride=8, act=_lib.ACT_GELU)
            if cfg.dconv_mode & 1:
                self._dconv(key, f"tencoder.{i}", y, B, Tout, 1, Cc, "_t")
            z = self._buf(key, f"saved_t{i}", B * tp(Tout) * Cc, zero=True)
            self._gemm(M=B * Tout, N=2 * Cc, Cin=Cc, x=y, w=W[f"tencoder.{i}.rewrite.w"],
                       bias=W[f"tencoder.{i}.rewrite.b"], out=z, act=_lib.ACT_GLU, I1=1, I0=Tout, J1=1, J0=Tout,
                       xs=(Tout * Cc, 0, Cc, 1), os_=(tp(Tout) * Cc, 0, Cc))
            saved_t.append(z)
            xt, Cin_t = z, Cc
            tap(f"tenc{i}", z.view(B, tp(Tout), Cc)[:, :Tout], "t")

            Fo = Fin // 4
            y = self._buf(key, "y_f", B * T * Fo * Cc)
            if conv0 and Cin == 4:
                self._k("bd_encoder_conv0", ptr(xf), 0, ptr(norm), 8, ptr(W[f"encoder.{i}.conv.w"]),
                        ptr(W[f"encoder.{i}.conv.b"]), ptr(y), B, T, Fo, Fin, Cin, Cc, self.thin_math, self._stream(),
                        flops=2.0 * B * T * Fo * Cc * 8 * Cin, nbytes=4.0 * B * T * (Fin * Cin + Fo * Cc),
                        label="encoder_conv0_mma", detail=f"M={B * T * Fo} cin={Cin}")
            else:
              self._gemm(M=B * T * Fo, N=Cc, Cin=Cin, x=xf, w=W[f"encoder.{i}.conv.w"], bias=W[f"encoder.{i}.conv.b"],
                       out=y, taps=tuple((0, k - 2) for k in range(8)), I1=T, I0=Fo, m0=4, J1=T, J0=Fin,
                       xs=(T * Fin * Cin, Fin * Cin, Cin, 1), os_=(T * Fo * Cc, Fo * Cc, Cc),
                       a_mode=_lib.A_ITEM_AFFINE if first else _lib.A_NONE,
                       a_stats=norm if first else None, a_stats_stride=8, act=_lib.ACT_GELU)
            if cfg.dconv_mode & 1:
                self._dconv(key, f"encoder.{i}", y, B, T, Fo, Cc, "_f")
            z = self._buf(key, f"saved_f{i}", B * T * Fo * Cc)
            emb = W["freq_emb"] if (first and cfg.freq_emb) else None
            self._gemm(M=B * T * Fo, N=2 * Cc, Cin=Cc, x=y, w=W[f"encoder.{i}.rewrite.w"],
                       bias=W[f"encoder.{i}.rewrite.b"], out=z, act=_lib.ACT_GLU,
                       rowbias=emb, rowbias_period=Fo if emb is not None else 0)
            saved.append(z)
            xf, Fin, Cin = z, Fo, Cc
            tap(f"enc{i}", z.view(B, T, Fo, Cc), "f")

        Fb, Cb, T2 = Fin, chans[-1], tl[-1]
        Mf, Mt = B * T * Fb, B * T2
        dec_f_numel = B * T * max(2048 * 4 * S, 512 * chans[0])
        dec_t_numel = B * max(tp(L) * 2 * S, tp(tl[1]) * chans[0])

        if cfg.t_layers > 0:
            D = cfg.transformer_dim
            if cfg.bottom_channels:
                x = self._buf(key, "tr_x", Mf * D)
                xt_ = self._buf(key, "tr_xt", Mt * D)
                self._gemm(M=Mf, N=D, Cin=Cb, x=xf, w=W["channel_upsampler.w"], bias=W["channel_upsampler.b"], out=x)
                self._gemm(M=Mt, N=D, Cin=Cb, x=xt, w=W["channel_upsampler_t.w"], bias=W["channel_upsampler_t.b"],
                           out=xt_, I1=1, I0=T2, J1=1, J0=T2, xs=(tp(T2) * Cb, 0, Cb, 1), os_=(T2 * D, 0, D))
            else:
                x = self._buf(key, "tr_x", Mf * D)
                xt_ = self._buf(key, "tr_xt", Mt * D)
                x.copy_(xf)
                xt_.view(B, T2, D).copy_(xt.view(B, tp(T2), Cb)[:, :T2])
            ct = "crosstransformer"
            pos2d = self._pos_table(("2d", Fb, T))
            pos1d = self._pos_table(("1d", T2))
            self._ln(x, x, f"{ct}.norm_in", Mf, pos2d, T * Fb)
            self._ln(xt_, xt_, f"{ct}.norm_in_t", Mt, pos1d, T2)
            for i in range(cfg.t_layers):
                if i % 2 == 0:
                    self._transformer_layer(key, x, None, f"{ct}.layers.{i}", False, B, T * Fb, T * Fb, "_f")
                    self._transformer_layer(key, xt_, None, f"{ct}.layers_t.{i}", False, B, T2, T2, "_t")
                else:
                    kdt = torch.bfloat16 if self.mode == "bf16" else torch.float32
                    kf = self._buf(key, "kn_f", Mt * D, kdt)
                    kt = self._buf(key, "kn_t", Mf * D, kdt)
                    self._ln(xt_, kf, f"{ct}.layers.{i}.norm2", Mt)
                    self._ln(x, kt, f"{ct}.layers_t.{i}.norm2", Mf)
                    self._transformer_layer(key, x, kf, f"{ct}.layers.{i}", True, B, T * Fb, T2, "_f")
                    self._transformer_layer(key, xt_, kt, f"{ct}.layers_t.{i}", True, B, T2, T * Fb, "_t")
                tap(f"xf.layer{i}", x.view(B, T, Fb, D), "f")
                tap(f"xt.layer{i}", xt_.view(B, T2, D), "t")
            xd = self._buf(key, "dec_a", dec_f_numel)[: Mf * Cb]
            xtd = self._buf(key, "dec_ta", dec_t_numel)[: B * tp(T2) * Cb]
            if cfg.bottom_channels:
                self._gemm(M=Mf, N=Cb, Cin=D, x=x, w=W["channel_downsampler.w"], bias=W["channel_downsampler.b"],
                           out=xd, addend=saved[-1])
                self._gemm(M=Mt, N=Cb, Cin=D, x=xt_, w=W["channel_downsampler_t.w"],
                           bias=W["channel_downsampler_t.b"], out=xtd, addend=saved_t[-1], I1=1, I0=T2, J1=1, J0=T2,
                           xs=(T2 * D, 0, D, 1), os_=(tp(T2) * Cb, 0, Cb))
            else:
                torch.add(x, saved[-1], out=xd)
                xtd.view(B, tp(T2), Cb)[:, :T2].copy_(xt_.view(B, T2, Cb) + saved_t[-1].view(B, tp(T2), Cb)[:, :T2])
            if taps is not None:
                tap("bottleneck", (xd - saved[-1]).view(B, T, Fb, Cb), "f")
                tap("bottleneck_t", (xtd - saved_t[-1]).view(B, tp(T2), Cb)[:, :T2], "t")
        else:
            xd = self._buf(key, "dec_a", dec_f_numel)[: Mf * Cb]
            xtd = self._buf(key, "dec_ta", dec_t_numel)[: B * tp(T2) * Cb]
            torch.add(xf, saved[-1], out=xd)
            torch.mul(saved_t[-1], 2.0, out=xtd)

        Fcur = Fb
        names = ("dec_a", "dec_b")
        for j in range(cfg.depth):
            Cc = chans[cfg.depth - 1 - j]
            last = j == cfg.depth - 1
            Cout = 4 * S if last else Cc // 2
            Cout_t = 2 * S if last else Cc // 2
            skip = None if last else saved[cfg.depth - 2 - j]
            skip_t = None if last else saved_t[cfg.depth - 2 - j]
            y = self._buf(key, "y_f", B * T * Fcur * Cc)
            taps9 = tuple((kt - 1, kf - 1) for kf in range(3) for kt in range(3))
            self._gemm(M=B * T * Fcur, N=2 * Cc, Cin=Cc, x=xd, w=W[f"decoder.{j}.rewrite.w"],
                       bias=W[f"decoder.{j}.rewrite.b"], out=y, taps=taps9, I1=T, I0=Fcur, J1=T, J0=Fcur,
                       xs=(T * Fcur * Cc, Fcur * Cc, Cc, 1), os_=(T * Fcur * Cc, Fcur * Cc, Cc), act=_lib.ACT_GLU)
            if cfg.dconv_mode & 2:
                self._dconv(key, f"decoder.{j}", y, B, T, Fcur, Cc, "_f")
            nxt = self._buf(key, names[(j + 1) % 2], dec_f_numel)[: B * T * 4 * Fcur * Cout]
            three = self.mode != "fp32" and 4 * Cout >= 64
            self._gemm(M=B * T * (Fcur + (0 if three else 1)), N=4 * Cout, Cin=Cc, x=y,
                       w=W[f"decoder.{j}.conv_tr.w3" if three else f"decoder.{j}.conv_tr.w"],
                       bias=W[f"decoder.{j}.conv_tr.b"], out=nxt,
                       taps=((0, -1), (0, 0), (0, 1)) if three else ((0, 0), (0, -1)), I1=T,
                       I0=Fcur + (0 if three else 1), J1=T, J0=Fcur, xs=(T * Fcur * Cc, Fcur * Cc, Cc, 1),
                       os_=(T * 4 * Fcur * Cout, 4 * Fcur * Cout, 4 if last else Cout),
                       oc_split=4 if last else 0, oc_stride=4 * Fcur * 4 if last else 0,
                       convt=2 if three else 1, O0=4 * Fcur,
                       act=_lib.ACT_NONE if last else _lib.ACT_GELU, addend=skip)
            if taps is not None:
                if last:
                    tap(f"dec{j}", nxt.view(B, T, S, 4 * Fcur, 4).permute(0, 1, 3, 2, 4).reshape(B, T, 4 * Fcur, Cout), "f")
                else:
                    tap(f"dec{j}", (nxt - skip).view(B, T, 4 * Fcur, Cout), "f")
            xd, Fcur = nxt, 4 * Fcur

            Tin, Tout = tl[cfg.depth - j], tl[cfg.depth - 1 - j]
            y = self._buf(key, "y_t", B * Tin * Cc)
            self._gemm(M=B * Tin, N=2 * Cc, Cin=Cc, x=xtd, w=W[f"tdecoder.{j}.rewrite.w"],
                       bias=W[f"tdecoder.{j}.rewrite.b"], out=y, taps=((0, -1), (0, 0), (0, 1)), I1=1, I0=Tin,
                       J1=1, J0=Tin, xs=(tp(Tin) * Cc, 0, Cc, 1), os_=(Tin * Cc, 0, Cc), act=_lib.ACT_GLU)
            if cfg.dconv_mode & 2:
                self._dconv(key, f"tdecoder.{j}", y, B, Tin, 1, Cc, "_t")
            nxt = self._buf(key, "dec_tb" if (j % 2 == 0) else "dec_ta", dec_t_numel)[: B * tp(Tout) * Cout_t]
            three = self.mode != "fp32" and 4 * Cout_t >= 64
            self._gemm(M=B * (Tin + (0 if three else 1)), N=4 * Cout_t, Cin=Cc, x=y,
                       w=W[f"tdecoder.{j}.conv_tr.w3" if three else f"tdecoder.{j}.conv_tr.w"],
                       bias=W[f"tdecoder.{j}.conv_tr.b"], out=nxt,
                       taps=((0, -1), (0, 0), (0, 1)) if three else ((0, 0), (0, -1)), I1=1,
                       I0=Tin + (0 if three else 1), J1=1, J0=Tin, xs=(Tin * Cc, 0, Cc, 1),
                       os_=(tp(Tout) * Cout_t, 0, Cout_t), convt=2 if three else 1, O0=Tout,
                       act=_lib.ACT_NONE if last else _lib.ACT_GELU, addend=skip_t)
            if taps is not None:
                tap(f"tdec{j}", (nxt - skip_t if skip_t is not None else nxt).view(B, tp(Tout), Cout_t)[:, :Tout], "t")
            xtd = nxt

        if mag is not None:
            nm = norm.view(B, 8)
            spec_out = xd[: B * T * S * 2048 * 2 * A].view(B, T, S, 2048, 2 * A).permute(0, 2, 4, 3, 1)
            spec_out = spec_out * nm[:, 1].view(B, 1, 1, 1, 1) + nm[:, 0].view(B, 1, 1, 1, 1)
            time_out = xtd[: B * tp(L) * A * S].view(B, tp(L), S, A)[:, :L].permute(0, 2, 3, 1)
            time_out = time_out * nm[:, 5].view(B, 1, 1, 1) + nm[:, 4].view(B, 1, 1, 1)
            return spec_out.contiguous(), time_out.contiguous()
        if out_buf is not None:
            if out_buf.numel() != B * S * A * L0 or out_buf.dtype != torch.float32 or out_buf.device != self.device \
                    or not out_buf.is_contiguous():
                raise ValueError("out must be a contiguous float32 tensor of B*S*C*L elements on the engine's device")
            out = out_buf.view(B, S, A, L0)
        else:
            out = torch.empty(B, S, A, L0, dtype=torch.float32, device=self.device)
        self._k("bd_istft_ola", ptr(xd), ptr(norm), ptr(self.window), ptr(self.twiddle), ptr(xtd), ptr(out),
                B, S, T, tp(L), L0, st, nbytes=4.0 * B * S * (T * 2048 * 4 + 2 * L + 2 * L0),
                flops=2.5 * 4096 * 12 * 2 * S * B * T)
        if taps is not None:
            only = torch.empty(B, S, A, L0, dtype=torch.float32, device=self.device)
            self._k("bd_istft_ola", ptr(xd), ptr(norm), ptr(self.window), ptr(self.twiddle), None, ptr(only),
                    B, S, T, tp(L), L0, st)
            taps["istft"] = only
            taps["time_out"] = out - only
        return out

    def _pos_table(self, key) -> torch.Tensor:
        t = self._pos.get(key)
        if t is None:
            cfg = self.cfg
            D = cfg.transformer_dim
            if key[0] == "2d":
                t = _sin_embedding_2d(D, key[1], key[2], cfg.t_max_period)
            else:
                t = _sin_embedding_1d(key[1], D, cfg.t_max_period)
            t = (cfg.t_weight_pos_embed * t).to(self.device).contiguous()
            self._pos[key] = t
        return t
```

Before: 2541.

## Add CTA-pair tcgen05 bf16x3 GEMM path with cost-model tile selection

Adds a 2-CTA cluster variant of the persistent conv GEMM that issues cta_group::2 tcgen05 MMAs over a 256-row M tile. Each CTA loads half of the B tile, and TMEM, barriers and commits are shared through the cluster. A simple cost model picks wide pair tiles (96/192/256) when it predicts fewer waves or less smem traffic per stage than the single-CTA tile. The aim is to halve per-CTA B operand loads and raise MMA efficiency for wide-N layers. In exchange it adds cluster synchronisation, cross-CTA mbarrier traffic and half as many scheduling slots.

```diff
diff --git a/demucs_b200/_lib.py b/demucs_b200/_lib.py
--- a/demucs_b200/_lib.py
+++ b/demucs_b200/_lib.py
@@ -8,7 +8,7 @@
 HERE = os.path.dirname(os.path.abspath(__file__))
 CSRC = os.path.join(HERE, "csrc")
 LIB_PATH = os.path.join(HERE, "libdemucs_b200.so")
-SOURCES = ["api.cu", "spectral.cu", "gemm_simt.cu", "gemm_tc.cu", "gemm_tc_b16x3.cu", "gemm_tc_b16.cu", "norm.cu", "dconv.cu", "attention.cu", "attention_tc.cu", "attention_b16.cu",
+SOURCES = ["api.cu", "spectral.cu", "gemm_simt.cu", "gemm_tc.cu", "gemm_tc_b16x3.cu", "gemm_tc_b16x3_pair.cu", "gemm_tc_b16.cu", "norm.cu", "dconv.cu", "attention.cu", "attention_tc.cu", "attention_b16.cu",
            "ola.cu", "audio.cu", "hdemucs.cu"]
 NVCC_FLAGS = ["-gencode", "arch=compute_100a,code=sm_100a", "-lineinfo", "-O3", "-std=c++17",
               "-Xcompiler", "-fPIC", "--use_fast_math=false"]
diff --git a/demucs_b200/csrc/gemm_tc.cu b/demucs_b200/csrc/gemm_tc.cu
--- a/demucs_b200/csrc/gemm_tc.cu
+++ b/demucs_b200/csrc/gemm_tc.cu
@@ -1,6 +1,7 @@
 #include "gemm_tc_impl.cuh"
 
 int bd_tc_launch_bf16x3(int tbk, int tbn, const bd_gemm_desc& d, const TileGeom& g, int items, cudaStream_t st);
+int bd_tc_launch_bf16x3_pair(int tbk, int tbn, const bd_gemm_desc& d, const TileGeom& g, int items, cudaStream_t st);
 int bd_tc_launch_bf16(int tbk, int tbn, const bd_gemm_desc& d, const TileGeom& g, int items, cudaStream_t st);
 int bd_tc_launch_bf16d(int tbk, int tbn, const bd_gemm_desc& d, const TileGeom& g, int items, cudaStream_t st);
 
@@ -45,6 +46,11 @@
   return g;
 }
 
+struct TileChoice {
+  int tbn;
+  bool pair;
+};
+
 int tile_width(const bd_gemm_desc& d, const TileGeom& g) {
   static const bool wide_ok = getenv("BD_TC_NO_WIDE") == nullptr;
   static const bool wide_x3 = getenv("BD_TC_NO_WIDE_X3") == nullptr;
@@ -60,6 +66,34 @@
   return d.N <= 16 ? 16 : d.N <= 32 ? 32 : d.N <= 64 ? 64 : 128;
 }
 
+double stage_clocks(int tbn, bool pair) {
+  const double c = pair ? tbn / 2 : tbn;
+  const double smem = (6.0 * (4096 + 32 * c) + 16384 + 128 * c + 32768) / 128.0;
+  return smem > 3.0 * tbn ? smem : 3.0 * tbn;
+}
+
+TileChoice tile_choice(const bd_gemm_desc& d, const TileGeom& g) {
+  const int tbn = tile_width(d, g);
+  if (d.math != BD_MATH_BF16X3 || getenv("BD_TC_NO_PAIR") != nullptr) return {tbn, false};
+  const long long rows = (long long)(d.M / (d.I0 * d.I1)) * g.blocks1 * g.blocks0;
+  auto cost = [&](int w, bool pair) {
+    const long long tiles = (pair ? (rows + 1) / 2 : rows) * ((d.N + w - 1) / w);
+    const int slots = pair ? 74 : 148;
+    return (double)((tiles + slots - 1) / slots) * stage_clocks(w, pair);
+  };
+  TileChoice best = {tbn, false};
+  double best_cost = cost(tbn, false);
+  for (int w : {256, 192, 96}) {
+    if (!(d.N % w == 0 && (w != 96 || d.N == 96))) continue;
+    const double c = cost(w, true);
+    if (c < best_cost) {
+      best = {w, true};
+      best_cost = c;
+    }
+  }
+  return best;
+}
+
 }
 
 static int k_block(const bd_gemm_desc& d, int tbn) {
@@ -70,8 +104,8 @@
 
 int bd_conv_gemm_tc_tile(const bd_gemm_desc& d) {
   if (!bd_conv_gemm_tc_eligible(d) || d.M % ((long long)d.I0 * d.I1) != 0) return 0;
-  const int tbn = tile_width(d, tile_geometry(d));
-  return 1000 * k_block(d, tbn) + tbn;
+  const TileChoice t = tile_choice(d, tile_geometry(d));
+  return 1000 * k_block(d, t.tbn) + t.tbn + (t.pair ? 500 : 0);
 }
 
 int bd_conv_gemm_tc(const bd_gemm_desc* dp, void* stream, int* handled) {
@@ -82,13 +116,16 @@
   BD_REQUIRE(d.M % ((long long)d.I0 * d.I1) == 0, "bd_conv_gemm: M not a multiple of I1*I0");
   TileGeom g = tile_geometry(d);
   const int items = d.M / (d.I0 * d.I1);
-  const int tbn = tile_width(d, g);
+  const TileChoice t = tile_choice(d, g);
+  const int tbn = t.tbn;
   const int tbk = k_block(d, tbn);
   g.cpb = d.Cin / tbk;
   const cudaStream_t st = (cudaStream_t)stream;
   int rc;
   switch (d.math) {
-    case BD_MATH_BF16X3: rc = bd_tc_launch_bf16x3(tbk, tbn, d, g, items, st); break;
+    case BD_MATH_BF16X3:
+      rc = t.pair ? bd_tc_launch_bf16x3_pair(tbk, tbn, d, g, items, st) : bd_tc_launch_bf16x3(tbk, tbn, d, g, items, st);
+      break;
     case BD_MATH_BF16:
       rc = d.x_bf16 ? bd_tc_launch_bf16d(tbk, tbn, d, g, items, st) : bd_tc_launch_bf16(tbk, tbn, d, g, items, st);
       break;
diff --git a/demucs_b200/csrc/gemm_tc_b16x3_pair.cu b/demucs_b200/csrc/gemm_tc_b16x3_pair.cu
--- /dev/null
+++ b/demucs_b200/csrc/gemm_tc_b16x3_pair.cu
@@ -0,0 +1,21 @@
+#include "gemm_tc_impl.cuh"
+
+int bd_tc_launch_bf16x3_pair(int tbk, int tbn, const bd_gemm_desc& d, const TileGeom& g, int items, cudaStream_t st) {
+  if (tbk == 32) {
+    switch (tbn) {
+      case 96: return launch_tc_persist<32, 96, BD_TC_BF16X3, true>(d, g, items, st);
+      case 192: return launch_tc_persist<32, 192, BD_TC_BF16X3, true>(d, g, items, st);
+      case 256: return launch_tc_persist<32, 256, BD_TC_BF16X3, true>(d, g, items, st);
+      default: break;
+    }
+  } else {
+    switch (tbn) {
+      case 96: return launch_tc_persist<16, 96, BD_TC_BF16X3, true>(d, g, items, st);
+      case 192: return launch_tc_persist<16, 192, BD_TC_BF16X3, true>(d, g, items, st);
+      case 256: return launch_tc_persist<16, 256, BD_TC_BF16X3, true>(d, g, items, st);
+      default: break;
+    }
+  }
+  bd_set_error("bd_conv_gemm_tc: no CTA-pair kernel for tile %d x %d", tbk, tbn);
+  return BD_ERR_ARG;
+}
diff --git a/demucs_b200/csrc/gemm_tc_impl.cuh b/demucs_b200/csrc/gemm_tc_impl.cuh
--- a/demucs_b200/csrc/gemm_tc_impl.cuh
+++ b/demucs_b200/csrc/gemm_tc_impl.cuh
@@ -107,6 +107,38 @@
   asm volatile("tcgen05.commit.cta_group::1.mbarrier::arrive::one.shared::cluster.b64 [%0];" ::"r"(smem_u32(bar))
                : "memory");
 }
+__device__ __forceinline__ void tcgen05_commit_pair(uint64_t* bar) {
+  asm volatile("tcgen05.commit.cta_group::2.mbarrier::arrive::one.shared::cluster.multicast::cluster.b64 [%0], %1;"
+               ::"r"(smem_u32(bar)), "h"((uint16_t)3)
+               : "memory");
+}
+__device__ __forceinline__ uint32_t cluster_ctarank() {
+  uint32_t r;
+  asm volatile("mov.u32 %0, %%cluster_ctarank;" : "=r"(r));
+  return r;
+}
+__device__ __forceinline__ void cluster_sync() {
+  asm volatile("barrier.cluster.arrive.release.aligned;\n\tbarrier.cluster.wait.acquire.aligned;" ::: "memory");
+}
+__device__ __forceinline__ void mbar_arrive_cta(uint64_t* bar, uint32_t rank) {
+  uint32_t a;
+  asm volatile("mapa.shared::cluster.u32 %0, %1, %2;" : "=r"(a) : "r"(smem_u32(bar)), "r"(rank));
+  asm volatile("mbarrier.arrive.release.cluster.shared::cluster.b64 _, [%0];" ::"r"(a) : "memory");
+}
+__device__ __forceinline__ void mbar_wait_parked_cluster(uint64_t* bar, uint32_t parity) {
+  uint32_t done = 0, spins = 0;
+  while (true) {
+    asm volatile(
+        "{\n\t.reg .pred p;\n\t"
+        "mbarrier.try_wait.parity.acquire.cluster.shared::cta.b64 p, [%1], %2, %3;\n\t"
+        "selp.u32 %0, 1, 0, p;\n\t}"
+        : "=r"(done)
+        : "r"(smem_u32(bar)), "r"(parity), "r"(1000)
+        : "memory");
+    if (done) return;
+    if (++spins > kSpinLimit) __trap();
+  }
+}
 __device__ __forceinline__ void tcgen05_fence_after() { asm volatile("tcgen05.fence::after_thread_sync;" ::: "memory"); }
 __device__ __forceinline__ void tcgen05_fence_before() { asm volatile("tcgen05.fence::before_thread_sync;" ::: "memory"); }
 
@@ -124,6 +156,15 @@
       "{\n\t.reg .pred p;\n\t"
       "setp.ne.b32 p, %4, 0;\n\t"
       "tcgen05.mma.cta_group::1.kind::f16 [%0], %1, %2, %3, p;\n\t}"
+      ::"r"(tmem_d), "l"(adesc), "l"(bdesc), "r"(idesc), "r"(accumulate)
+      : "memory");
+}
+__device__ __forceinline__ void umma_bf16_pair(uint32_t tmem_d, uint64_t adesc, uint64_t bdesc, uint32_t idesc,
+                                               uint32_t accumulate) {
+  asm volatile(
+      "{\n\t.reg .pred p;\n\t"
+      "setp.ne.b32 p, %4, 0;\n\t"
+      "tcgen05.mma.cta_group::2.kind::f16 [%0], %1, %2, %3, p;\n\t}"
       ::"r"(tmem_d), "l"(adesc), "l"(bdesc), "r"(idesc), "r"(accumulate)
       : "memory");
 }
@@ -203,9 +244,10 @@
   constexpr int LDT = WC + 4;
   constexpr int CG = WC / 4 < 32 ? WC / 4 : 32;
   constexpr int RPI = 32 / CG;
-  const int cg = lane % CG, rsub = lane / CG;
+  const bool lane_ok = CG * RPI == 32 || lane < CG * RPI;
+  const int cg = lane % CG, rsub = lane_ok ? lane / CG : 0;
   const int n = n0w + 4 * cg;
-  const bool col_ok = n < d.N;
+  const bool col_ok = n < d.N && lane_ok;
   const int nc = col_ok ? n : 0;
   const float4 bias = d.bias ? ldg4(d.bias + nc) : make_float4(0.f, 0.f, 0.f, 0.f);
   float4 gam = make_float4(1.f, 1.f, 1.f, 1.f), bet = make_float4(0.f, 0.f, 0.f, 0.f);
@@ -337,8 +379,10 @@
 #ifndef BD_TC_EPI_GROUPS
 #define BD_TC_EPI_GROUPS 4
 #endif
-template <int TBK, int TBN, int MODE>
+template <int TBK, int TBN, int MODE, bool PAIR = false>
 struct PCfg {
+  static_assert(!PAIR || MODE == BD_TC_BF16X3, "CTA pairs are built for the bf16x3 arithmetic only");
+  static constexpr int kBRows = PAIR ? TBN / 2 : TBN;
   static constexpr bool kX3 = MODE == BD_TC_TF32X3;
   static constexpr bool kB16 = MODE == BD_TC_BF16X3 || MODE == BD_TC_BF16 || MODE == BD_TC_BF16D;
   static constexpr bool kDirect = MODE == BD_TC_BF16D;
@@ -350,37 +394,42 @@
   static constexpr int kEpiWarp0 = kSplit ? kSplitWarp0 + kSplitWarps : 4;
   static constexpr int kThreads = 32 * kEpiWarp0 + 128 * kPGroups;
   static constexpr int kTileBytesA = TBM * TBK * (kDirect ? 2 : 4);
-  static constexpr int kTileBytesB = kB16 ? TBN * TBK * 2 : TBN * TBK * 4;
+  static constexpr int kTileBytesB = kB16 ? kBRows * TBK * 2 : kBRows * TBK * 4;
   static constexpr int kStageBytesA = (kX3 ? 2 : 1) * kTileBytesA;
   static constexpr int kStageBytesB = (kX3 ? 2 : kBParts) * kTileBytesB;
   static constexpr int kTxBytes = kTileBytesA + (kB16 ? kBParts : 1) * kTileBytesB;
   static constexpr bool kTileSplit = TBN <= 32;
   static constexpr int kNAcc = kTileSplit ? kPGroups : 2;
   static constexpr int kHalves = TBN > 128 ? 2 : 1;
-  static constexpr int kWarpCols = kTileSplit ? TBN : (TBN / kHalves) / kPGroups;
+  static constexpr int kHalfCols = TBN / kHalves;
+  static constexpr int kWarpCols = kTileSplit ? TBN : kHalfCols / kPGroups;
+  static_assert(kTileSplit || kWarpCols % 16 == 0, "epilogue warps read TMEM 16 or 32 columns at a time");
   static constexpr int kStagingBytes = 4 * kPGroups * 32 * (kWarpCols + 4) * 4;
   static constexpr int kTailBytes = 512 + 128 * kPGroups * 32;
   static constexpr int kBudget = 227 * 1024 - 1024 - kTailBytes - kStagingBytes;
   static constexpr int kStagesRaw = kBudget / (kStageBytesA + kStageBytesB);
   static constexpr int kStages = kStagesRaw > (kTileSplit ? 16 : 8) ? (kTileSplit ? 16 : 8) : kStagesRaw;
   static constexpr int kSmemBytes = kStages * (kStageBytesA + kStageBytesB) + kStagingBytes + 1024 + kTailBytes;
-  static constexpr int kTmemCols = kNAcc * TBN < 32 ? 32 : kNAcc * TBN;
+  static constexpr int kTmemCols = kNAcc * TBN <= 32 ? 32 : kNAcc * TBN <= 64 ? 64 : kNAcc * TBN <= 128 ? 128
+                                   : kNAcc * TBN <= 256 ? 256 : 512;
 };
 
-template <int TBK, int TBN, int MODE>
-__global__ void __launch_bounds__((PCfg<TBK, TBN, MODE>::kThreads), 1) conv_gemm_tc_persist_kernel(const __grid_constant__ CUtensorMap map_a,
+template <int TBK, int TBN, int MODE, bool PAIR = false>
+__global__ void __launch_bounds__((PCfg<TBK, TBN, MODE, PAIR>::kThreads), 1) conv_gemm_tc_persist_kernel(const __grid_constant__ CUtensorMap map_a,
                                                                             const __grid_constant__ CUtensorMap map_b,
                                                                             const __grid_constant__ CUtensorMap map_b_lo,
                                                                             const bd_gemm_desc d, const TileGeom g,
                                                                             int ntiles, int ntn) {
-  using C_ = PCfg<TBK, TBN, MODE>;
+  using C_ = PCfg<TBK, TBN, MODE, PAIR>;
   constexpr bool X3 = C_::kX3, B16 = C_::kB16, SPLIT = C_::kSplit;
   constexpr int kPGroups = C_::kPGroups;
   constexpr int kTileBytesA = C_::kTileBytesA, kTileBytesB = C_::kTileBytesB;
   constexpr int kStages = C_::kStages, kStageBytesA = C_::kStageBytesA, kStageBytesB = C_::kStageBytesB;
   constexpr int kTmemCols = C_::kTmemCols;
   constexpr int WC = C_::kWarpCols;
-  constexpr int CW = WC < 32 ? WC : 32;
+  constexpr int CW = WC % 32 == 0 ? 32 : 16;
+  constexpr int HC = C_::kHalfCols;
+  constexpr int kPeers = PAIR ? 2 : 1;
   extern __shared__ uint8_t smem_raw[];
   uint8_t* smem = reinterpret_cast<uint8_t*>(((uintptr_t)smem_raw + 1023) & ~(uintptr_t)1023);
   uint8_t* sA = smem;
@@ -398,32 +447,42 @@
 
   const int warp = threadIdx.x >> 5, lane = threadIdx.x & 31;
   const int nkb = d.taps * g.cpb;
+  const int rank = PAIR ? (int)cluster_ctarank() : 0;
+  const int first = PAIR ? (int)(blockIdx.x >> 1) : (int)blockIdx.x;
+  const int step = PAIR ? (int)(gridDim.x >> 1) : (int)gridDim.x;
 
   if (threadIdx.x == 0) {
     for (int s = 0; s < kStages; ++s) {
       mbar_init(&full_bar[s], 1);
       mbar_init(&empty_bar[s], 1);
-      mbar_init(&conv_bar[s], 32 * C_::kSplitWarps);
+      mbar_init(&conv_bar[s], 32 * C_::kSplitWarps * kPeers);
     }
     for (int a = 0; a < kNAcc; ++a) {
       mbar_init(&tmem_full[a], 1);
-      mbar_init(&tmem_empty[a], kTileSplit ? 4 : 4 * kPGroups);
+      mbar_init(&tmem_empty[a], (kTileSplit ? 4 : 4 * kPGroups) * kPeers);
     }
     asm volatile("fence.mbarrier_init.release.cluster;" ::: "memory");
   }
   if (warp == 1) {
-    asm volatile("tcgen05.alloc.cta_group::1.sync.aligned.shared::cta.b32 [%0], %1;" ::"r"(smem_u32(tmem_slot)),
-                 "r"(kTmemCols));
-    asm volatile("tcgen05.relinquish_alloc_permit.cta_group::1.sync.aligned;" ::);
+    if constexpr (PAIR) {
+      asm volatile("tcgen05.alloc.cta_group::2.sync.aligned.shared::cta.b32 [%0], %1;" ::"r"(smem_u32(tmem_slot)),
+                   "r"(kTmemCols));
+      asm volatile("tcgen05.relinquish_alloc_permit.cta_group::2.sync.aligned;" ::);
+    } else {
+      asm volatile("tcgen05.alloc.cta_group::1.sync.aligned.shared::cta.b32 [%0], %1;" ::"r"(smem_u32(tmem_slot)),
+                   "r"(kTmemCols));
+      asm volatile("tcgen05.relinquish_alloc_permit.cta_group::1.sync.aligned;" ::);
+    }
   }
   tcgen05_fence_before();
   __syncthreads();
+  if constexpr (PAIR) cluster_sync();
   tcgen05_fence_after();
   const uint32_t tmem_base = *tmem_slot;
 
   auto decode = [&](int tile, int& b, int& i0s, int& i1s, int& n0) {
     const int nb = tile % ntn;
-    int r = tile / ntn;
+    int r = PAIR ? 2 * (tile / ntn) + rank : tile / ntn;
     const int blk0 = r % g.blocks0;
     r /= g.blocks0;
     const int blk1 = r % g.blocks1;
@@ -436,9 +495,10 @@
   if (warp == 0) {
     if (lane == 0) {
       long long kbg = 0;
-      for (int tile = blockIdx.x; tile < ntiles; tile += gridDim.x) {
+      for (int tile = first; tile < ntiles; tile += step) {
         int b, i0s, i1s, n0;
         decode(tile, b, i0s, i1s, n0);
+        n0 += rank * C_::kBRows;
         int tap = 0, cb = 0;
         for (int kb = 0; kb < nkb; ++kb, ++kbg) {
           const int s = (int)(kbg % kStages);
@@ -462,19 +522,21 @@
       }
     }
   } else if (warp == 1) {
-    if (lane == 0) {
-      constexpr uint32_t idesc = B16 ? make_idesc_bf16(TBM, TBN) : make_idesc_tf32(TBM, TBN);
+    if (lane == 0 && rank == 0) {
+      constexpr uint32_t idesc = B16 ? make_idesc_bf16(TBM * kPeers, TBN) : make_idesc_tf32(TBM, TBN);
       long long kbg = 0;
       int tcount = 0;
-      for (int tile = blockIdx.x; tile < ntiles; tile += gridDim.x, ++tcount) {
+      for (int tile = first; tile < ntiles; tile += step, ++tcount) {
         const int a = tcount % kNAcc;
-        mbar_wait_parked(&tmem_empty[a], (uint32_t)(((tcount / kNAcc) & 1) ^ 1));
+        const uint32_t ea = (uint32_t)(((tcount / kNAcc) & 1) ^ 1);
+        if constexpr (PAIR) mbar_wait_parked_cluster(&tmem_empty[a], ea); else mbar_wait_parked(&tmem_empty[a], ea);
         tcgen05_fence_after();
         const uint32_t acc = tmem_base + (uint32_t)(a * TBN);
         for (int kb = 0; kb < nkb; ++kb, ++kbg) {
           const int s = (int)(kbg % kStages);
           const uint32_t ph = (uint32_t)((kbg / kStages) & 1);
-          mbar_wait_parked(SPLIT ? &conv_bar[s] : &full_bar[s], ph);
+          if constexpr (PAIR) mbar_wait_parked_cluster(&conv_bar[s], ph);
+          else mbar_wait_parked(SPLIT ? &conv_bar[s] : &full_bar[s], ph);
           tcgen05_fence_after();
           if constexpr (B16) {
             const uint64_t a_hi = make_kmajor_desc16<TBK>(sA + s * kStageBytesA, C_::kDirect ? 8 * TBK * 2 : 8 * TBK * 4);
@@ -483,7 +545,11 @@
             const uint64_t b_lo = make_kmajor_desc16<TBK>(sB + s * kStageBytesB + kTileBytesB, 8 * TBK * 2);
 #pragma unroll
             for (int k = 0; k < TBK / 16; ++k) {
-              if constexpr (MODE == BD_TC_BF16X3) {
+              if constexpr (PAIR) {
+                umma_bf16_pair(acc, a_lo + 2 * k, b_hi + 2 * k, idesc, (kb | k) != 0);
+                umma_bf16_pair(acc, a_hi + 2 * k, b_lo + 2 * k, idesc, 1);
+                umma_bf16_pair(acc, a_hi + 2 * k, b_hi + 2 * k, idesc, 1);
+              } else if constexpr (MODE == BD_TC_BF16X3) {
                 umma_bf16(acc, a_lo + 2 * k, b_hi + 2 * k, idesc, (kb | k) != 0);
                 umma_bf16(acc, a_hi + 2 * k, b_lo + 2 * k, idesc, 1);
                 umma_bf16(acc, a_hi + 2 * k, b_hi + 2 * k, idesc, 1);
@@ -507,9 +573,9 @@
             }
           }
           }
-          tcgen05_commit(&empty_bar[s]);
-        }
-        tcgen05_commit(&tmem_full[a]);
+          if constexpr (PAIR) tcgen05_commit_pair(&empty_bar[s]); else tcgen05_commit(&empty_bar[s]);
+        }
+        if constexpr (PAIR) tcgen05_commit_pair(&tmem_full[a]); else tcgen05_commit(&tmem_full[a]);
       }
     }
   } else if (SPLIT && warp >= C_::kSplitWarp0 && warp < C_::kSplitWarp0 + C_::kSplitWarps) {
@@ -524,7 +590,7 @@
       const int xin = (r * RB >> 7) & (RB / 16 - 1);
       const int xout = (r * RH >> 7) & (RH / 16 - 1);
       (void)et;
-      for (int tile = blockIdx.x; tile < ntiles; tile += gridDim.x) {
+      for (int tile = first; tile < ntiles; tile += step) {
         for (int kb = 0; kb < nkb; ++kb, ++kbg) {
           const int s = (int)(kbg % kStages);
           mbar_wait(&full_bar[s], (uint32_t)((kbg / kStages) & 1));
@@ -571,11 +637,11 @@
           }
           }
           asm volatile("fence.proxy.async.shared::cta;" ::: "memory");
-          mbar_arrive(&conv_bar[s]);
+          if constexpr (PAIR) mbar_arrive_cta(&conv_bar[s], 0); else mbar_arrive(&conv_bar[s]);
         }
       }
     } else {
-    for (int tile = blockIdx.x; tile < ntiles; tile += gridDim.x) {
+    for (int tile = first; tile < ntiles; tile += step) {
       for (int kb = 0; kb < nkb; ++kb, ++kbg) {
         const int s = (int)(kbg % kStages);
         mbar_wait(&full_bar[s], (uint32_t)((kbg / kStages) & 1));
@@ -606,16 +672,19 @@
     constexpr int LDT = WC + 4;
     float* stage = staging + (size_t)ew * 32 * LDT;
     RowInfo* rinfo = reinterpret_cast<RowInfo*>(((uintptr_t)(tmem_slot + 4) + 31) & ~(uintptr_t)31) + ew * 32;
+    auto arrive_tmem_empty = [&](int a) {
+      if constexpr (PAIR) mbar_arrive_cta(&tmem_empty[a], 0); else mbar_arrive(&tmem_empty[a]);
+    };
     int tcount = 0;
-    for (int tile = blockIdx.x; tile < ntiles; tile += gridDim.x, ++tcount) {
+    for (int tile = first; tile < ntiles; tile += step, ++tcount) {
       if (kTileSplit && tcount % kPGroups != grp) continue;
       int b, i0s, i1s, n0;
       decode(tile, b, i0s, i1s, n0);
       const int a = tcount % kNAcc;
       const int r = quarter * 32 + lane;
       const int i0 = i0s + (r & (g.R0 - 1)), i1 = i1s + (r >> g.log2R0);
-      const bool row_ok = i0 < d.I0 && i1 < d.I1;
       const long long m = ((long long)b * d.I1 + i1) * d.I0 + i0;
+      const bool row_ok = i0 < d.I0 && i1 < d.I1 && (!PAIR || m < d.M);
       EpiRow er;
       er.obase = 0; er.i0 = 0; er.rb_row = 0; er.e_mean = 0.f; er.e_rstd = 1.f;
       if (row_ok) {
@@ -639,7 +708,7 @@
         }
       }
       for (int half = 0; half < NH; ++half) {
-      const int n0h = n0 + 128 * half;
+      const int n0h = n0 + HC * half;
       if (half == 0) {
         mbar_wait_relaxed(&tmem_full[a], (uint32_t)((tcount / kNAcc) & 1));
         tcgen05_fence_after();
@@ -647,7 +716,7 @@
         __syncwarp();
       }
       const bool last_half = half == NH - 1;
-      const uint32_t acc = tmem_base + (uint32_t)(a * TBN + 128 * half + cbase) + ((uint32_t)(quarter * 32) << 16);
+      const uint32_t acc = tmem_base + (uint32_t)(a * TBN + HC * half + cbase) + ((uint32_t)(quarter * 32) << 16);
       if (vec) {
         rinfo[lane].obase = er.obase;
         rinfo[lane].i0 = row_ok ? er.i0 : -1;
@@ -666,7 +735,7 @@
         }
         tcgen05_fence_before();
         __syncwarp();
-        if (lane == 0 && last_half) mbar_arrive(&tmem_empty[a]);
+        if (lane == 0 && last_half) arrive_tmem_empty(a);
         if (fast >= 0) {
           const uint32_t st_s = smem_u32(stage), ri_s = smem_u32(rinfo);
           const int n0w = n0h + cbase;
@@ -685,9 +754,10 @@
         constexpr int CG = WC / 4 < 32 ? WC / 4 : 32;
         constexpr int RPI = 32 / CG;
         constexpr int RB = kPGroups >= 4 ? 2 : 4;
-        const int cg = lane % CG, rsub = lane / CG;
+        const bool lane_ok = CG * RPI == 32 || lane < CG * RPI;
+        const int cg = lane % CG, rsub = lane_ok ? lane / CG : 0;
         const int n = n0h + cbase + 4 * cg;
-        const bool col_ok = n < d.N;
+        const bool col_ok = n < d.N && lane_ok;
         EpiCol ecol;
         if (col_ok) ecol = bd_epi_cols4(d, n);
         for (int it = 0; it < 32 / RPI; it += RB) {
@@ -719,7 +789,7 @@
             }
             if (row_stats) {
               __syncwarp();
-              *reinterpret_cast<float2*>(stage + rloc * LDT + 2 * cg) = make_float2(rs, rq);
+              if (lane_ok) *reinterpret_cast<float2*>(stage + rloc * LDT + 2 * cg) = make_float2(rs, rq);
             } else {
               ssum += rs;
               ssq += rq;
@@ -763,7 +833,7 @@
         }
         tcgen05_fence_before();
         __syncwarp();
-        if (lane == 0 && last_half) mbar_arrive(&tmem_empty[a]);
+        if (lane == 0 && last_half) arrive_tmem_empty(a);
         if (row_stats && row_ok) {
           atomicAdd(&d.stats_out[2 * (size_t)my_slab], (double)ssum);
           atomicAdd(&d.stats_out[2 * (size_t)my_slab + 1], (double)ssq);
@@ -772,7 +842,7 @@
       }
       if (d.stats_out && d.stat_mod == 1) {
         const double ds = bd_warp_sum_d((double)ssum), dq = bd_warp_sum_d((double)ssq);
-        if (lane == 0) {
+        if (lane == 0 && (!PAIR || (long long)b * d.I1 * d.I0 < d.M)) {
           const int sl = bd_stat_slab(d, (long long)b * d.I1 * d.I0 + i0s);
           atomicAdd(&d.stats_out[2 * (size_t)sl], ds);
           atomicAdd(&d.stats_out[2 * (size_t)sl + 1], dq);
@@ -782,9 +852,13 @@
   }
   tcgen05_fence_before();
   __syncthreads();
+  if constexpr (PAIR) cluster_sync();
   if (warp == 1) {
     tcgen05_fence_after();
-    asm volatile("tcgen05.dealloc.cta_group::1.sync.aligned.b32 %0, %1;" ::"r"(tmem_base), "r"(kTmemCols));
+    if constexpr (PAIR)
+      asm volatile("tcgen05.dealloc.cta_group::2.sync.aligned.b32 %0, %1;" ::"r"(tmem_base), "r"(kTmemCols));
+    else
+      asm volatile("tcgen05.dealloc.cta_group::1.sync.aligned.b32 %0, %1;" ::"r"(tmem_base), "r"(kTmemCols));
   }
 }
 
@@ -817,9 +891,9 @@
              CU_TENSOR_MAP_FLOAT_OOB_FILL_NONE) == CUDA_SUCCESS;
 }
 
-template <int TBK, int TBN, int MODE>
+template <int TBK, int TBN, int MODE, bool PAIR = false>
 int launch_tc_persist(const bd_gemm_desc& d, const TileGeom& g, int items, cudaStream_t st) {
-  using C_ = PCfg<TBK, TBN, MODE>;
+  using C_ = PCfg<TBK, TBN, MODE, PAIR>;
   alignas(64) CUtensorMap map_a, map_b, map_b_lo;
   const long long s0 = d.xs_0, s1 = d.J1 > 1 ? d.xs_1 : s0 * d.J0, sb = items > 1 ? d.xs_b : s1 * d.J1;
   constexpr int ES = C_::kDirect ? 2 : 4;
@@ -834,7 +908,7 @@
     abox[1] = 1; abox[2] = (cuuint32_t)g.R0; abox[3] = (cuuint32_t)g.R1; abox[4] = 1;
   }
   cuuint64_t bdim[2] = {(cuuint64_t)d.K, (cuuint64_t)d.N};
-  cuuint32_t bbox[2] = {(cuuint32_t)TBK, (cuuint32_t)TBN};
+  cuuint32_t bbox[2] = {(cuuint32_t)TBK, (cuuint32_t)C_::kBRows};
   bool ok = encode(&map_a, d.x, arank, adim, astr, abox, TBK * ES, C_::kDirect);
   if constexpr (C_::kB16) {
     cuuint64_t bstr[1] = {(cuuint64_t)d.K * 2};
@@ -850,30 +924,57 @@
                  d.Cin, d.J0, d.J1);
     return BD_ERR_CUDA;
   }
-  static int sms_of[64] = {0};
+  auto kernel = conv_gemm_tc_persist_kernel<TBK, TBN, MODE, PAIR>;
+  static int slots_of[64] = {0};
   int dev = 0;
   cudaGetDevice(&dev);
   if (dev < 0 || dev >= 64) {
     bd_set_error("bd_conv_gemm_tc: device ordinal %d out of range", dev);
     return BD_ERR_ARG;
   }
-  if (!sms_of[dev]) {
-    cudaError_t e = cudaFuncSetAttribute(conv_gemm_tc_persist_kernel<TBK, TBN, MODE>,
-                                         cudaFuncAttributeMaxDynamicSharedMemorySize, C_::kSmemBytes);
+  cudaLaunchConfig_t cfg = {};
+  cudaLaunchAttribute attr[1];
+  cfg.blockDim = dim3(C_::kThreads);
+  cfg.dynamicSmemBytes = C_::kSmemBytes;
+  cfg.stream = st;
+  if (PAIR) {
+    attr[0].id = cudaLaunchAttributeClusterDimension;
+    attr[0].val.clusterDim.x = 2;
+    attr[0].val.clusterDim.y = 1;
+    attr[0].val.clusterDim.z = 1;
+    cfg.attrs = attr;
+    cfg.numAttrs = 1;
+  }
+  if (!slots_of[dev]) {
+    cudaError_t e = cudaFuncSetAttribute(kernel, cudaFuncAttributeMaxDynamicSharedMemorySize, C_::kSmemBytes);
     if (e != cudaSuccess) {
       bd_set_error("bd_conv_gemm_tc: cudaFuncSetAttribute: %s", cudaGetErrorString(e));
       return BD_ERR_CUDA;
     }
     int n = 0;
-    cudaDeviceGetAttribute(&n, cudaDevAttrMultiProcessorCount, dev);
-    sms_of[dev] = n;
-  }
-  const int sms = sms_of[dev];
+    if (PAIR) {
+      cfg.gridDim = dim3(2);
+      e = cudaOccupancyMaxActiveClusters(&n, kernel, &cfg);
+      if (e != cudaSuccess || n < 1) {
+        bd_set_error("bd_conv_gemm_tc: cudaOccupancyMaxActiveClusters: %s (%d clusters)", cudaGetErrorString(e), n);
+        return BD_ERR_CUDA;
+      }
+    } else {
+      cudaDeviceGetAttribute(&n, cudaDevAttrMultiProcessorCount, dev);
+    }
+    slots_of[dev] = n;
+  }
+  const int slots = slots_of[dev];
   const int ntn = (d.N + TBN - 1) / TBN;
-  const long long ntiles = (long long)items * g.blocks1 * g.blocks0 * ntn;
-  const int grid = (int)(ntiles < sms ? ntiles : sms);
-  conv_gemm_tc_persist_kernel<TBK, TBN, MODE><<<grid, C_::kThreads, C_::kSmemBytes, st>>>(map_a, map_b, map_b_lo, d, g,
-                                                                                         (int)ntiles, ntn);
+  const long long rows = (long long)items * g.blocks1 * g.blocks0;
+  const long long ntiles = (PAIR ? (rows + 1) / 2 : rows) * ntn;
+  const int grid = (int)(ntiles < slots ? ntiles : slots);
+  cfg.gridDim = dim3(grid * (PAIR ? 2 : 1));
+  cudaError_t e = cudaLaunchKernelEx(&cfg, kernel, map_a, map_b, map_b_lo, d, g, (int)ntiles, ntn);
+  if (e != cudaSuccess) {
+    bd_set_error("conv_gemm_tc_persist_kernel: launch: %s", cudaGetErrorString(e));
+    return BD_ERR_CUDA;
+  }
   return bd_check_launch("conv_gemm_tc_persist_kernel");
 }
 
diff --git a/demucs_b200/engine.py b/demucs_b200/engine.py
--- a/demucs_b200/engine.py
+++ b/demucs_b200/engine.py
@@ -267,7 +267,8 @@
         if d.math != _lib.MATH_FP32 and _lib.TEST_HOOK is None:
             code = _lib.lib().bd_conv_gemm_arm(C.byref(d))
             if code:
-                arm, tile = "tc", f"{code // 1000},{code % 1000}"
+                pair = code % 1000 >= 500
+                arm, tile = ("tc2" if pair else "tc"), f"{code // 1000},{code % 1000 - (500 if pair else 0)}"
         self._k("bd_conv_gemm", C.byref(d), self._stream(), flops=2.0 * M * N * K, nbytes=nbytes,
                 label=f"conv_gemm_{arm}<{tile}>",
                 detail=f"M={M} N={N} K={K} taps={len(taps)} act={act} a={a_mode} stats={int(stats_out is not None)}")
```

Result: slower. 2164, median of 6 (-14.8%).
